# CrystalSixone/VLN-MAGIC

Hardware: AMD Instinct MI355X
Metric: trajectory-steps/sec (whole node), MAGIC-S R2R pretrain (higher is better)
Workload: dtype bf16

## Files before the change

profiles/micro/chain_timing.hip:

```cpp
#include "../../vln-magic_amd/csrc/chain.hip"
#include <cstdio>
GroupState& group_state() { static thread_local GroupState g = {}; return g; }
static void* dmalloc(size_t n, int fill) { void* p; hipMalloc(&p, n); hipMemset(p, fill, n); return p; }
int main(int argc, char** argv) {
  const int M = argc > 1 ? atoi(argv[1]) : 3840;
  ChainParams P; memset(&P, 0, sizeof(P));
  P.M = M; P.ld_in = CH; P.Np = 3 * CH; P.eps = 1e-12f;
  P.in = dmalloc((size_t)M * CH * 2, 0x11); P.res = dmalloc((size_t)M * CH * 2, 0x11);
  P.Wa = dmalloc(CH * CH * 2, 0x11); P.ba = (float*)dmalloc(CH * 4, 0); P.g1 = (float*)dmalloc(CH * 4, 0x3c); P.b1 = (float*)dmalloc(CH * 4, 0);
  P.W1 = dmalloc(CI * CH * 2, 0x11); P.bi = (float*)dmalloc(CI * 4, 0); P.W2 = dmalloc(CI * CH * 2, 0x11); P.bo2 = (float*)dmalloc(CH * 4, 0);
  P.g2 = (float*)dmalloc(CH * 4, 0x3c); P.b2 = (float*)dmalloc(CH * 4, 0); P.y2 = dmalloc((size_t)M * CH * 2, 0);
  P.Wp = dmalloc(3 * CH * CH * 2, 0x11); P.bp = (float*)dmalloc(3 * CH * 4, 0); P.proj = dmalloc((size_t)M * 3 * CH * 2, 0);
  hipEvent_t e0, e1; hipEventCreate(&e0); hipEventCreate(&e1);
  for (int rows = 32; rows <= 64; rows += 32)
  for (int variant = 0; variant < 3; ++variant) {
    magic_chain_tile_rows(rows);
    ChainParams Q = P;
    if (variant == 1) { Q.Wp = nullptr; }
    if (variant == 2) { Q.W1 = nullptr; Q.Np = CH; Q.y1 = Q.y2; }
    for (int it = 0; it < 3; ++it) magic_chain_fwd(DT_BF16, &Q, sizeof(Q), nullptr);
    hipDeviceSynchronize();
    hipEventRecord(e0);
    for (int it = 0; it < 20; ++it) magic_chain_fwd(DT_BF16, &Q, sizeof(Q), nullptr);
    hipEventRecord(e1); hipEventSynchronize(e1);
    float ms; hipEventElapsedTime(&ms, e0, e1);
    long long t[16]; hipMemcpyFromSymbol(t, HIP_SYMBOL(chain_ticks), sizeof(t));
    if (rows == 64) {
      printf("M %d rows 64 variant %d: %.1f us per launch; tile 0 (10 ns ticks): prologue %lld, stage-1 products %lld, LayerNorm 1 %lld, FFN (4 chunks) %lld, LayerNorm 2 %lld, y2 store + projection %lld, total %lld\n",
             M, variant, ms * 1000 / 20, t[1] - t[0], t[7] - t[1], t[2] - t[7], t[3] - t[2], t[4] - t[3], t[6] - t[4], t[6] - t[0]);
      continue;
    }
    printf("M %d variant %d (%s): %.1f us per launch; tile 0 (10 ns ticks): rows+params+ring prologue %lld, stage 1 %lld, 2a (8 chunks) %lld, 2b (8 chunks + LN) %lld, y2 store + 3 %lld, tail %lld, total %lld\n",
           M, variant, variant == 0 ? "full" : variant == 1 ? "no projection" : "mini", ms * 1000 / 20,
           t[1] - t[0], t[2] - t[1], t[3] - t[2], t[4] - t[3], t[5] - t[4], t[6] - t[5], t[6] - t[0]);
  }
  return 0;
}
```

vln-magic_amd/csrc/chain.hip:

```cpp
#include "enc_common.hpp"
#include "group.hpp"
#include <cstdlib>

#define CH 256
#define CI 1024
#define KP 264
#define KG 1032
#define CADDR(row, col, pitch) ((row) * (pitch) + (col))
#define CP 264
#define CG 1032

using ChainParams = magic_chain_params;

#define CRT 2
#define CROWS (16 * CRT)
#ifndef CNB
#define CNB 3
#endif

template <typename Hh>
__device__ __forceinline__ void chain_norm(f32x4 (&acc)[CRT][2], const float* sPar, const Hh* sR,
                                           float* red, Hh* sOut, const int nq, const float eps, const int w, const int lane) {
  const int g = lane >> 4, c16 = lane & 15;
  float bv[2], gv[2], btv[2];
#pragma unroll
  for (int ct = 0; ct < 2; ++ct) {
    const int col = (2 * w + ct) * 16 + c16;
    bv[ct] = sPar[col]; gv[ct] = sPar[CH + col]; btv[ct] = sPar[2 * CH + col];
  }
  float s[CRT][4];
#pragma unroll
  for (int rt = 0; rt < CRT; ++rt)
#pragma unroll
    for (int r = 0; r < 4; ++r) {
      const int row = rt * 16 + 4 * g + r;
#pragma unroll
      for (int ct = 0; ct < 2; ++ct) acc[rt][ct][r] += bv[ct] + to_f(sR[CADDR(row, (2 * w + ct) * 16 + c16, KP)]);
      s[rt][r] = row16_sum(acc[rt][0][r] + acc[rt][1][r]);
    }
  if (c16 == 0) {
#pragma unroll
    for (int rt = 0; rt < CRT; ++rt)
#pragma unroll
      for (int r = 0; r < 4; ++r) red[w * CROWS + rt * 16 + 4 * g + r] = s[rt][r];
  }
  __syncthreads();
  float mean[CRT][4];
#pragma unroll
  for (int rt = 0; rt < CRT; ++rt)
#pragma unroll
    for (int r = 0; r < 4; ++r) {
      float t = 0.f;
#pragma unroll
      for (int ww = 0; ww < NWAVE; ++ww) t += red[ww * CROWS + rt * 16 + 4 * g + r];
      mean[rt][r] = t * (1.0f / CH);
      const float d0 = acc[rt][0][r] - mean[rt][r], d1 = acc[rt][1][r] - mean[rt][r];
      s[rt][r] = row16_sum(d0 * d0 + d1 * d1);
    }
  if (c16 == 0) {
#pragma unroll
    for (int rt = 0; rt < CRT; ++rt)
#pragma unroll
      for (int r = 0; r < 4; ++r) red[NWAVE * CROWS + w * CROWS + rt * 16 + 4 * g + r] = s[rt][r];
  }
  __syncthreads();
#pragma unroll
  for (int rt = 0; rt < CRT; ++rt)
#pragma unroll
    for (int r = 0; r < 4; ++r) {
      const int rr = rt * 16 + 4 * g + r;
      float t = 0.f;
#pragma unroll
      for (int ww = 0; ww < NWAVE; ++ww) t += red[NWAVE * CROWS + ww * CROWS + rr];
      const float rstd = rsqrtf(t * (1.0f / CH) + eps);
#pragma unroll
      for (int ct = 0; ct < 2; ++ct)
        sOut[CADDR(rr, (2 * w + ct) * 16 + c16, KP)] = (rr < nq) ? from_f<Hh>((acc[rt][ct][r] - mean[rt][r]) * rstd * gv[ct] + btv[ct]) : (Hh)0.0f;
    }
}

template <typename Hh>
__device__ __forceinline__ void chain_rows_in(const Hh* src, long long ld, int nq, Hh* dst, int tid) {
  typedef __attribute__((ext_vector_type(4))) unsigned u4;
  for (int id = tid; id < CROWS * (CH / 8); id += NWAVE * 64) {
    const int r = id / (CH / 8), c = (id % (CH / 8)) * 8;
    const u4 v = r < nq ? *(const u4*)(src + r * ld + c) : (u4){0u, 0u, 0u, 0u};
    *(u4*)(dst + CADDR(r, c, KP)) = v;
  }
}

template <typename Hh> __device__ __forceinline__ h16x8<Hh> pfrag(const Hh* __restrict__ Wf, const int K, const int nt, const int ks, const int lane) {
  return *(const h16x8<Hh>*)(Wf + ((long long)(nt * (K >> 5) + ks) * 64 + lane) * 8);
}

template <typename Hh>
__device__ __forceinline__ void chain_load_chunk(h16x8<Hh> (&b)[8], const int cid, const ChainParams& p, const int w, const int lane, const int nct) {
  if (cid < 2) {
#pragma unroll
    for (int ks = 0; ks < 8; ++ks) b[ks] = pfrag((const Hh*)p.Wa, CH, 2 * w + cid, ks, lane);
  } else if (cid < 10) {
#pragma unroll
    for (int ks = 0; ks < 8; ++ks) b[ks] = pfrag((const Hh*)p.W1, CH, 8 * w + cid - 2, ks, lane);
  } else if (cid < 18) {
#pragma unroll
    for (int ks = 0; ks < 4; ++ks) {
      b[ks] = pfrag((const Hh*)p.W2, CI, 2 * w, 4 * (cid - 10) + ks, lane);
      b[4 + ks] = pfrag((const Hh*)p.W2, CI, 2 * w + 1, 4 * (cid - 10) + ks, lane);
    }
  } else {
    const Hh* Wq = p.Wp ? (const Hh*)p.Wp : (const Hh*)p.Wa;
    const int j = cid - 18, nt = p.Wp ? w * nct + (j < nct ? j : nct - 1) : 2 * w;
#pragma unroll
    for (int ks = 0; ks < 8; ++ks) b[ks] = pfrag(Wq, CH, nt, ks, lane);
  }
}

#ifdef CHAIN_TIMING
__device__ long long chain_ticks[16];
#define CH_MARK(i) do { if (tile == 0 && tid == 0) chain_ticks[i] = wall_clock64(); } while (0)
#else
#define CH_MARK(i)
#endif
template <typename Hh, bool FFN>
__device__ __forceinline__ void chain_body(const ChainParams& p, const int tile, unsigned char* smem) {
  Hh* sIn = (Hh*)smem;
  Hh* sRes = sIn + CROWS * KP;
  Hh* sY1 = sRes + CROWS * KP;
  Hh* sG = sY1 + CROWS * KP;
  float* red = (float*)(sG + CROWS * KG);
  Hh* sProj = sG;
  float* sPar = red + 2 * NWAVE * CROWS;
  const int tid = threadIdx.x, lane0 = tid & 63, w = __builtin_amdgcn_readfirstlane(tid >> 6);
  int lane = lane0;
  asm volatile("" : "+v"(lane));
  const int g = lane >> 4, c16 = lane & 15;
  const int row0 = tile * CROWS, nq = min(CROWS, p.M - row0);
  const int nct = p.Wp ? (p.Np >> 7) : 0;
  constexpr int NS = FFN ? 24 : 8;
#define SEQ(s) (FFN ? (s) : ((s) < 2 ? (s) : (s) + 16))
#define AHEAD(s) do { if ((s) + CNB - 1 < NS) chain_load_chunk<Hh>(ring[((s) + CNB - 1) % CNB], SEQ((s) + CNB - 1), p, w, lane, nct); } while (0)
  CH_MARK(0);
  chain_rows_in((const Hh*)p.inp + (long long)row0 * p.ld_in, p.ld_in, nq, sIn, tid);
  chain_rows_in((const Hh*)p.res + (long long)row0 * CH, CH, nq, sRes, tid);
  if (tid < CH) {
    sPar[tid] = p.ba[tid]; sPar[CH + tid] = p.g1[tid]; sPar[2 * CH + tid] = p.b1[tid];
    if (FFN) { sPar[3 * CH + tid] = p.bo2[tid]; sPar[4 * CH + tid] = p.g2[tid]; sPar[5 * CH + tid] = p.b2[tid]; }
  }
  if (FFN) { sPar[6 * CH + tid] = p.bi[tid]; sPar[6 * CH + 512 + tid] = p.bi[512 + tid]; }
  for (int i = tid; i < nct * 128; i += NWAVE * 64) sPar[6 * CH + CI + i] = p.bp[i];
  h16x8<Hh> ring[CNB][8];
#pragma unroll
  for (int s = 0; s < CNB - 1; ++s) chain_load_chunk<Hh>(ring[s], SEQ(s), p, w, lane, nct);
  __syncthreads();
  CH_MARK(1);
  {
    f32x4 acc[CRT][2];
#pragma unroll
    for (int rt = 0; rt < CRT; ++rt) { acc[rt][0] = (f32x4){0.f, 0.f, 0.f, 0.f}; acc[rt][1] = (f32x4){0.f, 0.f, 0.f, 0.f}; }
#pragma unroll
    for (int i = 0; i < 2; ++i) {
      AHEAD(i);
      KSTEP_FENCE();
#pragma unroll
      for (int ks = 0; ks < 8; ++ks)
#pragma unroll
        for (int rt = 0; rt < CRT; ++rt) acc[rt][i] = mfma16(frag_kc(sIn, KP, rt * 16, ks * 32, lane), ring[i % CNB][ks], acc[rt][i]);
      KSTEP_FENCE();
    }
    chain_norm(acc, sPar, sRes, red, sY1, nq, p.eps, w, lane);
  }
  __syncthreads();
  CH_MARK(2);
  if (p.y1) copy_out(sY1, KP, (Hh*)p.y1 + (long long)row0 * CH, CH, nq, CH, tid);
  const Hh* sLast = sY1;
  if constexpr (FFN) {
    {
#pragma unroll
      for (int ct = 0; ct < 8; ++ct) {
        AHEAD(2 + ct);
        const int col = (8 * w + ct) * 16 + c16;
        const float bfc = sPar[6 * CH + col];
        KSTEP_FENCE();
        f32x4 acc[CRT];
#pragma unroll
        for (int rt = 0; rt < CRT; ++rt) acc[rt] = (f32x4){0.f, 0.f, 0.f, 0.f};
#pragma unroll
        for (int ks = 0; ks < 8; ++ks)
#pragma unroll
          for (int rt = 0; rt < CRT; ++rt) acc[rt] = mfma16(frag_kc(sY1, KP, rt * 16, ks * 32, lane), ring[(2 + ct) % CNB][ks], acc[rt]);
#pragma unroll
        for (int rt = 0; rt < CRT; ++rt)
#pragma unroll
          for (int r = 0; r < 4; ++r) sG[CADDR(rt * 16 + 4 * g + r, col, KG)] = from_f<Hh>(gelu_fast(acc[rt][r] + bfc));
        KSTEP_FENCE();
      }
    }
    __syncthreads();
    CH_MARK(3);
    {
      f32x4 acc[CRT][2];
#pragma unroll
      for (int rt = 0; rt < CRT; ++rt) { acc[rt][0] = (f32x4){0.f, 0.f, 0.f, 0.f}; acc[rt][1] = (f32x4){0.f, 0.f, 0.f, 0.f}; }
#pragma unroll
      for (int ch = 0; ch < 8; ++ch) {
        AHEAD(10 + ch);
        KSTEP_FENCE();
#pragma unroll
        for (int ks = 0; ks < 4; ++ks)
#pragma unroll
          for (int rt = 0; rt < CRT; ++rt) {
            const h16x8<Hh> a = frag_kc(sG, KG, rt * 16, (4 * ch + ks) * 32, lane);
            acc[rt][0] = mfma16(a, ring[(10 + ch) % CNB][ks], acc[rt][0]);
            acc[rt][1] = mfma16(a, ring[(10 + ch) % CNB][4 + ks], acc[rt][1]);
          }
        KSTEP_FENCE();
      }
      chain_norm(acc, sPar + 3 * CH, sY1, red, sIn, nq, p.eps, w, lane);
    }
    __syncthreads();
    CH_MARK(4);
    copy_out(sIn, KP, (Hh*)p.y2 + (long long)row0 * CH, CH, nq, CH, tid);
    sLast = sIn;
  }
  if (nct) {
    constexpr int S3 = FFN ? 18 : 2;
    const int pp = p.Np + 8;
#pragma unroll
    for (int j = 0; j < 6; ++j) {
      AHEAD(S3 + j);
      if (j < nct) {
        const int tile_n = w * nct + j;
        const float bpv = sPar[6 * CH + CI + tile_n * 16 + c16];
        KSTEP_FENCE();
        f32x4 acc[CRT];
#pragma unroll
        for (int rt = 0; rt < CRT; ++rt) acc[rt] = (f32x4){0.f, 0.f, 0.f, 0.f};
#pragma unroll
        for (int ks = 0; ks < 8; ++ks)
#pragma unroll
          for (int rt = 0; rt < CRT; ++rt) acc[rt] = mfma16(frag_kc(sLast, KP, rt * 16, ks * 32, lane), ring[(S3 + j) % CNB][ks], acc[rt]);
#pragma unroll
        for (int rt = 0; rt < CRT; ++rt)
#pragma unroll
          for (int r = 0; r < 4; ++r) sProj[(rt * 16 + 4 * g + r) * pp + tile_n * 16 + c16] = from_f<Hh>(acc[rt][r] + bpv);
      }
      KSTEP_FENCE();
    }
    __syncthreads();
    CH_MARK(5);
    copy_out(sProj, pp, (Hh*)p.proj + (long long)row0 * p.Np, p.Np, nq, p.Np, tid);
  }
  CH_MARK(6);
#undef SEQ
#undef AHEAD
}

struct ChainPair { ChainParams p[2]; int split; };
#ifndef CHAIN_ATTR
#define CHAIN_ATTR
#endif
template <typename Hh>
__global__ __launch_bounds__(512) CHAIN_ATTR void chain_fwd_kernel(ChainPair pr) {
  extern __shared__ __attribute__((aligned(16))) unsigned char chain_smem[];
  const int which = (int)blockIdx.x < pr.split ? 0 : 1;
  const ChainParams& p = pr.p[which];
  const int tile = which ? blockIdx.x - pr.split : blockIdx.x;
  if (p.W1) chain_body<Hh, true>(p, tile, chain_smem);
  else chain_body<Hh, false>(p, tile, chain_smem);
}


typedef __attribute__((ext_vector_type(16))) float f32x16;
__device__ __forceinline__ f32x16 mfma32(bf16x8 a, bf16x8 b, f32x16 c) { return __builtin_amdgcn_mfma_f32_32x32x16_bf16(a, b, c, 0, 0, 0); }
__device__ __forceinline__ f32x16 mfma32(f16x8 a, f16x8 b, f32x16 c) { return __builtin_amdgcn_mfma_f32_32x32x16_f16(a, b, c, 0, 0, 0); }
template <typename Hh> __device__ __forceinline__ h16x8<Hh> lfrag32(const Hh* s, int pitch, int row0, int k0, int lane) {
  return *(const h16x8<Hh>*)(s + (row0 + (lane & 31)) * pitch + k0 + 8 * (lane >> 5));
}
template <typename Hh> __device__ __forceinline__ h16x8<Hh> pfrag32(const Hh* __restrict__ Wf, const int K, const int NT, const int KS, const int lane) {
  const int nt16 = 2 * NT + ((lane >> 4) & 1), l2 = (lane & 15) + 16 * (2 * (KS & 1) + (lane >> 5));
  return *(const h16x8<Hh>*)(Wf + ((long long)(nt16 * (K >> 5) + (KS >> 1)) * 64 + l2) * 8);
}
#define C6ROWS 64
#define C6RT 2
#define C6NB 3
template <typename Hh>
__device__ __forceinline__ void chain64_load_chunk(h16x8<Hh> (&b)[8], const int cid, const ChainParams& p, const int w, const int lane, const int nj) {
  if (cid < 2) {
#pragma unroll
    for (int ks = 0; ks < 8; ++ks) b[ks] = pfrag32((const Hh*)p.Wa, CH, w, 8 * cid + ks, lane);
  } else if (cid < 18) {
    const int c = (cid - 2) >> 2, q = (cid - 2) & 3;
    if (q < 2) {
#pragma unroll
      for (int ks = 0; ks < 8; ++ks) b[ks] = pfrag32((const Hh*)p.W1, CH, 8 * c + w, 8 * q + ks, lane);
    } else {
#pragma unroll
      for (int ks = 0; ks < 8; ++ks) b[ks] = pfrag32((const Hh*)p.W2, CI, w, 16 * c + 8 * (q - 2) + ks, lane);
    }
  } else {
    const Hh* Wq = p.Wp ? (const Hh*)p.Wp : (const Hh*)p.Wa;
    const int j = (cid - 18) >> 1, hf = (cid - 18) & 1, nt = p.Wp ? 8 * (j < nj ? j : nj - 1) + w : w;
#pragma unroll
    for (int ks = 0; ks < 8; ++ks) b[ks] = pfrag32(Wq, CH, nt, 8 * hf + ks, lane);
  }
}
template <typename Hh>
__device__ __forceinline__ void chain64_norm(f32x16 (&acc)[C6RT], const float* sPar, const Hh* sR, float* red, Hh* sOut, const float eps,
                                             const int w, const int lane) {
  const int col = 32 * w + (lane & 31), h = lane >> 5, sub = (lane >> 4) & 1;
  const float bv = sPar[col], gv = sPar[CH + col], btv = sPar[2 * CH + col];
  float* part1 = red;
  float* part2 = red + 16 * C6ROWS;
  float* stat = red + 32 * C6ROWS + w * C6ROWS;
#pragma unroll
  for (int rt = 0; rt < C6RT; ++rt)
#pragma unroll
    for (int i = 0; i < 16; ++i) {
      const int row = rt * 32 + (i & 3) + 8 * (i >> 2) + 4 * h;
      acc[rt][i] += bv + to_f(sR[row * CP + col]);
      const float s = row16_sum(acc[rt][i]);
      if ((lane & 15) == 0) part1[(2 * w + sub) * C6ROWS + row] = s;
    }
  __syncthreads();
  {
    float t = 0.f;
#pragma unroll
    for (int q = 0; q < 16; ++q) t += part1[q * C6ROWS + lane];
    stat[lane] = t * (1.0f / CH);
  }
  wave_lds_sync();
#pragma unroll
  for (int rt = 0; rt < C6RT; ++rt)
#pragma unroll
    for (int i4 = 0; i4 < 4; ++i4) {
      const f32x4 m4 = *(const f32x4*)(stat + rt * 32 + 8 * i4 + 4 * h);
#pragma unroll
      for (int r = 0; r < 4; ++r) {
        const int i = 4 * i4 + r, row = rt * 32 + r + 8 * i4 + 4 * h;
        acc[rt][i] -= m4[r];
        const float s = row16_sum(acc[rt][i] * acc[rt][i]);
        if ((lane & 15) == 0) part2[(2 * w + sub) * C6ROWS + row] = s;
      }
    }
  __syncthreads();
  {
    float t = 0.f;
#pragma unroll
    for (int q = 0; q < 16; ++q) t += part2[q * C6ROWS + lane];
    wave_lds_sync();
    stat[lane] = rsqrtf(t * (1.0f / CH) + eps);
  }
  wave_lds_sync();
#pragma unroll
  for (int rt = 0; rt < C6RT; ++rt)
#pragma unroll
    for (int i4 = 0; i4 < 4; ++i4) {
      const f32x4 r4 = *(const f32x4*)(stat + rt * 32 + 8 * i4 + 4 * h);
#pragma unroll
      for (int r = 0; r < 4; ++r) {
        const int i = 4 * i4 + r, row = rt * 32 + r + 8 * i4 + 4 * h;
        sOut[row * CP + col] = from_f<Hh>(acc[rt][i] * r4[r] * gv + btv);
      }
    }
}
template <typename Hh>
__device__ __forceinline__ void chain64_rows_in(const Hh* src, long long ld, int nq, Hh* dst, int tid) {
  typedef __attribute__((ext_vector_type(4))) unsigned u4;
  for (int id = tid; id < C6ROWS * (CH / 8); id += NWAVE * 64) {
    const int r = id / (CH / 8), c = (id % (CH / 8)) * 8;
    const u4 v = r < nq ? *(const u4*)(src + r * ld + c) : (u4){0u, 0u, 0u, 0u};
    *(u4*)(dst + r * CP + c) = v;
  }
}
template <typename Hh, bool FFN>
__device__ __forceinline__ void chain64_body(const ChainParams& p, const int tile, unsigned char* smem) {
  Hh* sIn = (Hh*)smem;
  Hh* sRes = sIn + C6ROWS * CP;
  Hh* sY1 = sRes + C6ROWS * CP;
  Hh* sG = sY1 + C6ROWS * CP;
  float* red = (float*)(sG + C6ROWS * CP);
  float* sPar = red + 40 * C6ROWS;
  const int tid = threadIdx.x, lane0 = tid & 63, w = __builtin_amdgcn_readfirstlane(tid >> 6);
  int lane = lane0;
  asm volatile("" : "+v"(lane));
  const int h = lane >> 5, c32 = lane & 31;
  const int row0 = tile * C6ROWS, nq = min(C6ROWS, p.M - row0);
  const int nj = p.Wp ? (p.Np >> 8) : 0;
  constexpr int NS = FFN ? 24 : 8;
#define SEQ6(s) (FFN ? (s) : ((s) < 2 ? (s) : (s) + 16))
#define AHEAD6(s) do { if ((s) + C6NB - 1 < NS) chain64_load_chunk<Hh>(ring[((s) + C6NB - 1) % C6NB], SEQ6((s) + C6NB - 1), p, w, lane, nj); } while (0)
  CH_MARK(0);
  chain64_rows_in((const Hh*)p.inp + (long long)row0 * p.ld_in, p.ld_in, nq, sIn, tid);
  chain64_rows_in((const Hh*)p.res + (long long)row0 * CH, CH, nq, sRes, tid);
  if (tid < CH) {
    sPar[tid] = p.ba[tid]; sPar[CH + tid] = p.g1[tid]; sPar[2 * CH + tid] = p.b1[tid];
    if (FFN) { sPar[3 * CH + tid] = p.bo2[tid]; sPar[4 * CH + tid] = p.g2[tid]; sPar[5 * CH + tid] = p.b2[tid]; }
  }
  if (FFN) { sPar[6 * CH + tid] = p.bi[tid]; sPar[6 * CH + 512 + tid] = p.bi[512 + tid]; }
  for (int i = tid; i < nj * 256; i += NWAVE * 64) sPar[6 * CH + CI + i] = p.bp[i];
  h16x8<Hh> ring[C6NB][8];
#pragma unroll
  for (int s = 0; s < C6NB - 1; ++s) chain64_load_chunk<Hh>(ring[s], SEQ6(s), p, w, lane, nj);
  __syncthreads();
  CH_MARK(1);
  {
    f32x16 acc[C6RT];
#pragma unroll
    for (int rt = 0; rt < C6RT; ++rt)
#pragma unroll
      for (int i = 0; i < 16; ++i) acc[rt][i] = 0.f;
#pragma unroll
    for (int i = 0; i < 2; ++i) {
      AHEAD6(i);
      KSTEP_FENCE();
#pragma unroll
      for (int ks = 0; ks < 8; ++ks)
#pragma unroll
        for (int rt = 0; rt < C6RT; ++rt) acc[rt] = mfma32(lfrag32(sIn, CP, rt * 32, (8 * i + ks) * 16, lane), ring[i % C6NB][ks], acc[rt]);
      KSTEP_FENCE();
    }
    CH_MARK(7);
    chain64_norm(acc, sPar, sRes, red, sY1, p.eps, w, lane);
  }
  __syncthreads();
  CH_MARK(2);
  if (p.y1) copy_out(sY1, CP, (Hh*)p.y1 + (long long)row0 * CH, CH, nq, CH, tid);
  const Hh* sLast = sY1;
  if constexpr (FFN) {
    f32x16 acc2[C6RT];
#pragma unroll
    for (int rt = 0; rt < C6RT; ++rt)
#pragma unroll
      for (int i = 0; i < 16; ++i) acc2[rt][i] = 0.f;
#pragma unroll
    for (int c = 0; c < 4; ++c) {
      Hh* gbuf = (c & 1) ? sRes : sG;
      {
        f32x16 acc[C6RT];
#pragma unroll
        for (int rt = 0; rt < C6RT; ++rt)
#pragma unroll
          for (int i = 0; i < 16; ++i) acc[rt][i] = 0.f;
        const float bfc = sPar[6 * CH + 256 * c + 32 * w + c32];
#pragma unroll
        for (int q = 0; q < 2; ++q) {
          AHEAD6(2 + 4 * c + q);
          KSTEP_FENCE();
#pragma unroll
          for (int ks = 0; ks < 8; ++ks)
#pragma unroll
            for (int rt = 0; rt < C6RT; ++rt) acc[rt] = mfma32(lfrag32(sY1, CP, rt * 32, (8 * q + ks) * 16, lane), ring[(2 + 4 * c + q) % C6NB][ks], acc[rt]);
          KSTEP_FENCE();
        }
#pragma unroll
        for (int rt = 0; rt < C6RT; ++rt)
#pragma unroll
          for (int i = 0; i < 16; ++i)
            gbuf[(rt * 32 + (i & 3) + 8 * (i >> 2) + 4 * h) * CP + 32 * w + c32] = from_f<Hh>(gelu_fast(acc[rt][i] + bfc));
      }
      __syncthreads();
#pragma unroll
      for (int q = 0; q < 2; ++q) {
        AHEAD6(4 + 4 * c + q);
        KSTEP_FENCE();
#pragma unroll
        for (int ks = 0; ks < 8; ++ks)
#pragma unroll
          for (int rt = 0; rt < C6RT; ++rt) acc2[rt] = mfma32(lfrag32(gbuf, CP, rt * 32, (8 * q + ks) * 16, lane), ring[(4 + 4 * c + q) % C6NB][ks], acc2[rt]);
        KSTEP_FENCE();
      }
    }
    CH_MARK(3);
    chain64_norm(acc2, sPar + 3 * CH, sY1, red, sIn, p.eps, w, lane);
    __syncthreads();
    CH_MARK(4);
    copy_out(sIn, CP, (Hh*)p.y2 + (long long)row0 * CH, CH, nq, CH, tid);
    sLast = sIn;
  }
  if (nj) {
    constexpr int S3 = FFN ? 18 : 2;
#pragma unroll
    for (int j = 0; j < 3; ++j) {
      f32x16 acc[C6RT];
#pragma unroll
      for (int rt = 0; rt < C6RT; ++rt)
#pragma unroll
        for (int i = 0; i < 16; ++i) acc[rt][i] = 0.f;
#pragma unroll
      for (int q = 0; q < 2; ++q) {
        AHEAD6(S3 + 2 * j + q);
        KSTEP_FENCE();
        if (j < nj) {
#pragma unroll
          for (int ks = 0; ks < 8; ++ks)
#pragma unroll
            for (int rt = 0; rt < C6RT; ++rt) acc[rt] = mfma32(lfrag32(sLast, CP, rt * 32, (8 * q + ks) * 16, lane), ring[(S3 + 2 * j + q) % C6NB][ks], acc[rt]);
        }
        KSTEP_FENCE();
      }
      if (j < nj) {
        const float bpv = sPar[6 * CH + CI + 256 * j + 32 * w + c32];
        Hh* pbuf = (j & 1) ? sRes : sG;
#pragma unroll
        for (int rt = 0; rt < C6RT; ++rt)
#pragma unroll
          for (int i = 0; i < 16; ++i)
            pbuf[(rt * 32 + (i & 3) + 8 * (i >> 2) + 4 * h) * CP + 32 * w + c32] = from_f<Hh>(acc[rt][i] + bpv);
        __syncthreads();
        copy_out(pbuf, CP, (Hh*)p.proj + (long long)row0 * p.Np + 256 * j, p.Np, nq, 256, tid);
      }
    }
  }
  CH_MARK(6);
#undef SEQ6
#undef AHEAD6
}
template <typename Hh>
__global__ __launch_bounds__(512) void chain64_fwd_kernel(ChainPair pr) {
  extern __shared__ __attribute__((aligned(16))) unsigned char chain_smem[];
  const int which = (int)blockIdx.x < pr.split ? 0 : 1;
  const ChainParams& p = pr.p[which];
  const int tile = which ? blockIdx.x - pr.split : blockIdx.x;
  if (p.W1) chain64_body<Hh, true>(p, tile, chain_smem);
  else chain64_body<Hh, false>(p, tile, chain_smem);
}
static size_t chain64_lds_bytes() { return (size_t)(4 * C6ROWS * CP) * 2 + (40 * C6ROWS + 6 * CH + CI + 3 * CH) * sizeof(float); }

static size_t chain_lds_bytes() { return (size_t)(3 * CROWS * KP + CROWS * KG) * 2 + (2 * NWAVE * CROWS + 6 * CH + CI + 3 * CH) * sizeof(float); }

static bool chain_valid(const ChainParams& p) {
  if (p.M <= 0 || !p.inp || !p.res || !p.Wa || !p.ba || !p.g1 || !p.b1 || p.ld_in < CH || (p.ld_in & 7)) return false;
  if (p.W1 && (!p.bi || !p.W2 || !p.bo2 || !p.g2 || !p.b2 || !p.y2)) return false;
  if (p.Wp && (!p.bp || !p.proj || (p.Np != CH && p.Np != 2 * CH && p.Np != 3 * CH))) return false;
  if (!p.W1 && !p.y1 && !p.Wp) return false;
  return true;
}

static int chain_rows_cfg = 0;
extern "C" int magic_chain_tile_rows(int rows) {
  if (!chain_rows_cfg) { const char* e = getenv("MAGIC_CHAIN_ROWS"); const int v = e ? atoi(e) : 1; chain_rows_cfg = (v == 32 || v == 64) ? v : 1; }
  if (rows == 1 || rows == 32 || rows == 64) chain_rows_cfg = rows;
  else if (rows != 0) return MAGIC_ERR_ARG;
  return chain_rows_cfg;
}

int launch_chain(int dtype, int variant, const void* pa_, const void* pb_, hipStream_t st) {
  (void)variant;
  ChainPair pr;
  pr.p[0] = *(const ChainParams*)pa_;
  pr.p[1] = pb_ ? *(const ChainParams*)pb_ : pr.p[0];
  static int min_tiles = -1;
  if (min_tiles < 0) {
    const char* e = getenv("MAGIC_CHAIN_64_MIN_TILES");
    hipDeviceProp_t pr; int d = 0; (void)hipGetDevice(&d);
    min_tiles = e ? atoi(e) : ((hipGetDeviceProperties(&pr, d) == hipSuccess ? pr.multiProcessorCount : 256) + 1);
  }
  const int t32 = (pr.p[0].M + 31) / 32 + (pb_ ? (pr.p[1].M + 31) / 32 : 0);
  const int cfg = magic_chain_tile_rows(0);
  const int rows = cfg == 1 ? (t32 >= min_tiles ? 64 : 32) : cfg;
  const int ta = (pr.p[0].M + rows - 1) / rows, tb = pb_ ? (pr.p[1].M + rows - 1) / rows : 0;
  pr.split = ta;
  static bool attr_done[3] = {false, false, false};
  if (!attr_done[dtype == DT_BF16 ? DT_BF16 : DT_F16]) {
    DISPATCH_H(dtype, hipFuncSetAttribute((const void*)chain_fwd_kernel<TY>, hipFuncAttributeMaxDynamicSharedMemorySize, (int)chain_lds_bytes());
                      hipFuncSetAttribute((const void*)chain64_fwd_kernel<TY>, hipFuncAttributeMaxDynamicSharedMemorySize, (int)chain64_lds_bytes()));
    attr_done[dtype == DT_BF16 ? DT_BF16 : DT_F16] = true;
  }
  const size_t lds = rows == 64 ? chain64_lds_bytes() : chain_lds_bytes();
  DISPATCH_H(dtype, if (rows == 64) hipLaunchKernelGGL(chain64_fwd_kernel<TY>, dim3(ta + tb), dim3(512), lds, st, pr);
                    else hipLaunchKernelGGL(chain_fwd_kernel<TY>, dim3(ta + tb), dim3(512), lds, st, pr));
  return launch_status();
}

#define FSP_MAX 160
struct FSpans { long long off[FSP_MAX]; int rows[FSP_MAX]; int cols[FSP_MAX]; int blk0[FSP_MAX + 1]; int n; };
__global__ __launch_bounds__(256) void pack_frag_spans_kernel(const unsigned short* __restrict__ src, unsigned short* __restrict__ dst, FSpans t) {
  typedef __attribute__((ext_vector_type(8))) unsigned short u16x8;
  const int id = blockIdx.x;
  int s = 0;
  for (int i = 1; i < t.n; ++i) s += (id >= t.blk0[i]) ? 1 : 0;
  const int C = t.cols[s];
  const long long chunk = (long long)(id - t.blk0[s]) * 256 + threadIdx.x;
  const int l = (int)(chunk & 63);
  const long long frag = chunk >> 6;
  const int kpr = C >> 5, nt = (int)(frag / kpr), ks = (int)(frag % kpr);
  const unsigned short* a = src + t.off[s] + (long long)(16 * nt + (l & 15)) * C + 32 * ks + 8 * (l >> 4);
  *(u16x8*)(dst + t.off[s] + chunk * 8) = *(const u16x8*)a;
}
extern "C" int magic_pack_frag_spans(const void* src, void* dst, int n, const long long* offs, const int* rows, const int* cols, void* stream) {
  if (!src || !dst || n < 0 || (n && (!offs || !rows || !cols)) || ((uintptr_t)src & 15) || ((uintptr_t)dst & 15)) return MAGIC_ERR_ARG;
  for (int i = 0; i < n; ++i)
    if (rows[i] <= 0 || cols[i] <= 0 || rows[i] % 16 || cols[i] % 32 || ((long long)rows[i] * cols[i]) % 2048 || offs[i] % 8) return MAGIC_ERR_ARG;
  for (int base = 0; base < n; base += FSP_MAX) {
    FSpans t;
    t.n = n - base < FSP_MAX ? n - base : FSP_MAX;
    int blocks = 0;
    for (int i = 0; i < t.n; ++i) {
      t.off[i] = offs[base + i]; t.rows[i] = rows[base + i]; t.cols[i] = cols[base + i];
      t.blk0[i] = blocks;
      blocks += (int)(((long long)rows[base + i] * cols[base + i]) / 2048);
    }
    t.blk0[t.n] = blocks;
    hipLaunchKernelGGL(pack_frag_spans_kernel, dim3(blocks), dim3(256), 0, (hipStream_t)stream, (const unsigned short*)src, (unsigned short*)dst, t);
  }
  return launch_status();
}

struct LSpans { long long off[FSP_MAX]; int rows[FSP_MAX]; int cols[FSP_MAX]; int flags[FSP_MAX]; int tile0[FSP_MAX + 1]; int n; };
__global__ __launch_bounds__(256) void layout_spans_kernel(const unsigned short* __restrict__ src, unsigned short* __restrict__ dst_f,
                                                           unsigned short* __restrict__ dst_tf, LSpans t) {
  typedef __attribute__((ext_vector_type(8))) unsigned short u16x8;
  __shared__ unsigned short tile[64][72];
  const int id = blockIdx.x;
  int s = 0;
  for (int i = 1; i < t.n; ++i) s += (id >= t.tile0[i]) ? 1 : 0;
  const int local = id - t.tile0[s], R = t.rows[s], C = t.cols[s], fl = t.flags[s];
  const int tc = C / 64, r0 = (local / tc) * 64, c0 = (local % tc) * 64;
  const unsigned short* a = src + t.off[s];
#pragma unroll
  for (int it = 0; it < 2; ++it) {
    const int ch = threadIdx.x + it * 256, r = ch >> 3, c = (ch & 7) * 8;
    const u16x8 v = *(const u16x8*)(a + (long long)(r0 + r) * C + c0 + c);
    *(u16x8*)&tile[r][c] = v;
    if (fl & 1) {
      const int nt = (r0 + r) >> 4, rr = (r0 + r) & 15, ks = (c0 + c) >> 5, g = ((c0 + c) & 31) >> 3;
      *(u16x8*)(dst_f + t.off[s] + ((long long)(nt * (C >> 5) + ks) * 64 + g * 16 + rr) * 8) = v;
    }
  }
  if (!(fl & 2)) return;
  __syncthreads();
#pragma unroll
  for (int it = 0; it < 2; ++it) {
    const int ch = threadIdx.x + it * 256, l = ch & 63, fr = ch >> 6, i = fr >> 1, j = fr & 1, g = l >> 4, nn = l & 15;
    u16x8 v;
#pragma unroll
    for (int e = 0; e < 8; ++e) v[e] = tile[32 * j + 8 * g + e][16 * i + nn];
    const int nt = (c0 >> 4) + i, ks = (r0 >> 5) + j;
    *(u16x8*)(dst_tf + t.off[s] + ((long long)(nt * (R >> 5) + ks) * 64 + l) * 8) = v;
  }
}
extern "C" int magic_layout_spans(const void* src, void* dst_f, void* dst_tf, int n, const long long* offs, const int* rows, const int* cols,
                                  const int* flags, void* stream) {
  if (!src || n < 0 || (n && (!offs || !rows || !cols || !flags)) || ((uintptr_t)src & 15) || ((uintptr_t)dst_f & 15) || ((uintptr_t)dst_tf & 15)) return MAGIC_ERR_ARG;
  for (int i = 0; i < n; ++i) {
    if (rows[i] <= 0 || cols[i] <= 0 || rows[i] % 64 || cols[i] % 64 || offs[i] % 8 || !(flags[i] & 3)) return MAGIC_ERR_ARG;
    if (((flags[i] & 1) && !dst_f) || ((flags[i] & 2) && !dst_tf)) return MAGIC_ERR_ARG;
  }
  for (int base = 0; base < n; base += FSP_MAX) {
    LSpans t;
    t.n = n - base < FSP_MAX ? n - base : FSP_MAX;
    int tiles = 0;
    for (int i = 0; i < t.n; ++i) {
      t.off[i] = offs[base + i]; t.rows[i] = rows[base + i]; t.cols[i] = cols[base + i]; t.flags[i] = flags[base + i];
      t.tile0[i] = tiles;
      tiles += (rows[base + i] / 64) * (cols[base + i] / 64);
    }
    t.tile0[t.n] = tiles;
    hipLaunchKernelGGL(layout_spans_kernel, dim3(tiles), dim3(256), 0, (hipStream_t)stream, (const unsigned short*)src, (unsigned short*)dst_f,
                       (unsigned short*)dst_tf, t);
  }
  return launch_status();
}

extern "C" int magic_chain_supported(int dtype, int H, int I) { return dtype_is16(dtype) && H == CH && I == CI; }

extern "C" int magic_chain_fwd(int dtype, const void* params, int nbytes, void* stream) {
  if (!params || nbytes != (int)sizeof(ChainParams) || !dtype_is16(dtype)) return MAGIC_ERR_ARG;
  ChainParams p;
  memcpy(&p, params, sizeof(p));
  if (!chain_valid(p)) return MAGIC_ERR_ARG;
  if (group_record(KIND_CHAIN, dtype, 0, &p, sizeof(p))) return MAGIC_OK;
  return launch_chain(dtype, 0, &p, nullptr, (hipStream_t)stream);
}
```

vln-magic_amd/csrc/common.hpp:

```cpp
#pragma once
#include <hip/hip_runtime.h>
#include <stdint.h>
#include "../../include/magic_hip.h"

typedef __bf16 bf16;
typedef __attribute__((ext_vector_type(8))) __bf16 bf16x8;
typedef __attribute__((ext_vector_type(4))) __bf16 bf16x4;
typedef __attribute__((ext_vector_type(4))) float f32x4;
typedef _Float16 f16;
typedef __attribute__((ext_vector_type(8))) _Float16 f16x8;
typedef __attribute__((ext_vector_type(4))) _Float16 f16x4;
typedef __attribute__((ext_vector_type(4))) short s16x4;

#define DT_F32 0
#define DT_BF16 1
#define DT_F16 2
static inline bool dtype_ok(int dt) { return dt == DT_F32 || dt == DT_BF16 || dt == DT_F16; }
static inline bool dtype_is16(int dt) { return dt == DT_BF16 || dt == DT_F16; }

#define DISPATCH_T(dtype, ...)                                                        \
  do {                                                                                \
    if ((dtype) == DT_BF16) { typedef bf16 TY; __VA_ARGS__; }                          \
    else if ((dtype) == DT_F16) { typedef f16 TY; __VA_ARGS__; }                       \
    else { typedef float TY; __VA_ARGS__; }                                           \
  } while (0)
#define DISPATCH_H(dtype, ...)                                                        \
  do {                                                                                \
    if ((dtype) == DT_BF16) { typedef bf16 TY; __VA_ARGS__; }                          \
    else { typedef f16 TY; __VA_ARGS__; }                                             \
  } while (0)
#define DISPATCH_NIT(dtype, H, F)                                                                                       \
  DISPATCH_T(dtype, if ((H) == 128) F(TY, 1); else if ((H) == 256) F(TY, 2); else if ((H) == 384) F(TY, 3);              \
                    else if ((H) == 768) F(TY, 6); else return MAGIC_ERR_UNSUPPORTED)
#define DISPATCH_I2(v, A, B, ...)                                                     \
  do {                                                                                \
    if ((v) == (A)) { constexpr int IV = (A); __VA_ARGS__; }                           \
    else { constexpr int IV = (B); __VA_ARGS__; }                                     \
  } while (0)
#define DISPATCH_I3(v, A, B, C, ...)                                                  \
  do {                                                                                \
    if ((v) == (A)) { constexpr int IV = (A); __VA_ARGS__; }                           \
    else if ((v) == (B)) { constexpr int IV = (B); __VA_ARGS__; }                      \
    else { constexpr int IV = (C); __VA_ARGS__; }                                     \
  } while (0)

#define WAVE 64

__device__ __forceinline__ float to_f(float x) { return x; }
__device__ __forceinline__ float to_f(bf16 x) { return (float)x; }
__device__ __forceinline__ float to_f(f16 x) { return (float)x; }
template <typename T> __device__ __forceinline__ T from_f(float x);
template <> __device__ __forceinline__ float from_f<float>(float x) { return x; }
template <> __device__ __forceinline__ bf16 from_f<bf16>(float x) { return (bf16)x; }
template <> __device__ __forceinline__ f16 from_f<f16>(float x) { return (f16)x; }

template <typename Hh> struct H16;
template <> struct H16<bf16> { typedef bf16x8 v8; typedef bf16x4 v4; };
template <> struct H16<f16> { typedef f16x8 v8; typedef f16x4 v4; };
template <typename Hh> using h16x8 = typename H16<Hh>::v8;
template <typename Hh> using h16x4 = typename H16<Hh>::v4;
__device__ __forceinline__ f32x4 mfma16(bf16x8 a, bf16x8 b, f32x4 c) { return __builtin_amdgcn_mfma_f32_16x16x32_bf16(a, b, c, 0, 0, 0); }
__device__ __forceinline__ f32x4 mfma16(f16x8 a, f16x8 b, f32x4 c) { return __builtin_amdgcn_mfma_f32_16x16x32_f16(a, b, c, 0, 0, 0); }
__device__ __forceinline__ bf16x4 lds_tr4(const bf16* p) {
  typedef bf16x4 __attribute__((address_space(3))) * lds4;
  return __builtin_amdgcn_ds_read_tr16_b64_v4bf16((lds4)p);
}
__device__ __forceinline__ f16x4 lds_tr4(const f16* p) {
  typedef s16x4 __attribute__((address_space(3))) * lds4;
  return __builtin_bit_cast(f16x4, __builtin_amdgcn_ds_read_tr16_b64_v4i16((lds4)p));
}
template <typename Hh> __device__ __forceinline__ h16x8<Hh> lds_tr8(const Hh* p, int pitch4) {
  const h16x4<Hh> lo = lds_tr4(p), hi = lds_tr4(p + pitch4);
  return __builtin_shufflevector(lo, hi, 0, 1, 2, 3, 4, 5, 6, 7);
}
__device__ __forceinline__ f32x4 mfma16(float a, float b, f32x4 c) { return __builtin_amdgcn_mfma_f32_16x16x4f32(a, b, c, 0, 0, 0); }
template <typename Hh> __device__ __forceinline__ h16x8<Hh> frag_kc(const Hh* s, int pitch, int row0, int k0, int lane) {
  return *(const h16x8<Hh>*)(s + (row0 + (lane & 15)) * pitch + k0 + 8 * (lane >> 4));
}
template <typename Hh> __device__ __forceinline__ h16x8<Hh> frag_oc(const Hh* s, int pitch, int row0, int k0, int lane) {
  const int g = lane >> 4, q = (lane & 15) >> 2, pp = lane & 3;
  return lds_tr8(s + (k0 + 8 * g + q) * pitch + row0 + 4 * pp, 4 * pitch);
}
__device__ __forceinline__ float frag_kc(const float* s, int pitch, int row0, int k0, int lane) { return s[(row0 + (lane & 15)) * pitch + k0 + (lane >> 4)]; }
__device__ __forceinline__ float frag_oc(const float* s, int pitch, int row0, int k0, int lane) { return s[(k0 + (lane >> 4)) * pitch + row0 + (lane & 15)]; }

template <typename T> struct RowVecT { typedef T type __attribute__((ext_vector_type(16 / sizeof(T)))); };
template <typename T> using rowvec = typename RowVecT<T>::type;
template <typename T> struct RowImg {
  T* s; int pitch;
  const T* src; int ld;
  int nvalid, cvalid;
  int cpr, nchunk;
};
template <int NIT, typename T>
__device__ __forceinline__ void stage_issue(rowvec<T> (&reg)[NIT], const RowImg<T>& im, const int it0, const int tid, const int nthr) {
  constexpr int VE = 16 / sizeof(T);
#pragma unroll
  for (int it = 0; it < NIT; ++it) {
    const int id = tid + (it0 + it) * nthr, r = id / im.cpr, c = (id - r * im.cpr) * VE;
#pragma unroll
    for (int e = 0; e < VE; ++e) reg[it][e] = (T)0.0f;
    if (id < im.nchunk && r < im.nvalid && c < im.cvalid) reg[it] = *(const rowvec<T>*)(im.src + c + __mul24(r, im.ld));
  }
}
template <int NIT, typename T>
__device__ __forceinline__ void stage_store(const rowvec<T> (&reg)[NIT], const RowImg<T>& im, const int it0, const int tid, const int nthr) {
  constexpr int VE = 16 / sizeof(T);
#pragma unroll
  for (int it = 0; it < NIT; ++it) {
    const int id = tid + (it0 + it) * nthr, r = id / im.cpr, c = (id - r * im.cpr) * VE;
    if (id < im.nchunk) *(rowvec<T>*)(im.s + r * im.pitch + c) = reg[it];
  }
}

template <int CTRL> __device__ __forceinline__ float dpp_mov(float v) {
  return __int_as_float(__builtin_amdgcn_update_dpp(0, __float_as_int(v), CTRL, 0xF, 0xF, true));
}
#define DPP_QUAD_XOR1 0xB1
#define DPP_QUAD_XOR2 0x4E
#define DPP_ROW_HALF_MIRROR 0x141
#define DPP_ROW_MIRROR 0x140
__device__ __forceinline__ float row16_sum(float v) {
  v += dpp_mov<DPP_QUAD_XOR1>(v);
  v += dpp_mov<DPP_QUAD_XOR2>(v);
  v += dpp_mov<DPP_ROW_HALF_MIRROR>(v);
  v += dpp_mov<DPP_ROW_MIRROR>(v);
  return v;
}
__device__ __forceinline__ float row16_max(float v) {
  v = fmaxf(v, dpp_mov<DPP_QUAD_XOR1>(v));
  v = fmaxf(v, dpp_mov<DPP_QUAD_XOR2>(v));
  v = fmaxf(v, dpp_mov<DPP_ROW_HALF_MIRROR>(v));
  v = fmaxf(v, dpp_mov<DPP_ROW_MIRROR>(v));
  return v;
}
__device__ __forceinline__ float lane_bcast(float v, int lane) { return __int_as_float(__builtin_amdgcn_readlane(__float_as_int(v), lane)); }
__device__ __forceinline__ float wave_sum(float v) {
  v = row16_sum(v);
  return (lane_bcast(v, 0) + lane_bcast(v, 16)) + (lane_bcast(v, 32) + lane_bcast(v, 48));
}
__device__ __forceinline__ float wave_max(float v) {
  v = row16_max(v);
  return fmaxf(fmaxf(lane_bcast(v, 0), lane_bcast(v, 16)), fmaxf(lane_bcast(v, 32), lane_bcast(v, 48)));
}
__device__ __forceinline__ int wave_min_i(int v) {
#pragma unroll
  for (int d = 1; d < WAVE; d <<= 1) v = min(v, __shfl_xor(v, d));
  return v;
}
template <typename T> __device__ __forceinline__ T wave_scan_sum(T v, int lane) {
#pragma unroll
  for (int d = 1; d < WAVE; d <<= 1) {
    const T o = __shfl_up(v, d);
    if (lane >= d) v += o;
  }
  return v;
}

__device__ __forceinline__ float gelu_f(float x) { return 0.5f * x * (1.0f + erff(x * 0.70710678118654752f)); }
__device__ __forceinline__ float dgelu_f(float x) {
  float cdf = 0.5f * (1.0f + erff(x * 0.70710678118654752f));
  float pdf = 0.39894228040143268f * __expf(-0.5f * x * x);
  return cdf + x * pdf;
}

using DropDesc = magic_drop_desc;
struct DropState { unsigned ka, kb, thr; float scale; bool on; };
__device__ __forceinline__ DropState drop_init(const DropDesc& d) {
  DropState s;
  s.on = d.seed != nullptr && d.p > 0.f;
  s.ka = 0; s.kb = 0; s.thr = 0; s.scale = 1.f;
  if (s.on) {
    s.ka = d.seed[0] ^ (d.site * 0x9E3779B1u);
    s.kb = d.seed[1] + d.site * 0x85EBCA77u;
    s.thr = (unsigned)((double)d.p * 4294967296.0);
    s.scale = 1.0f / (1.0f - d.p);
  }
  return s;
}
__device__ __forceinline__ float drop_mul(const DropState& s, unsigned idx) {
  unsigned x = (idx ^ s.ka) + s.kb;
  x ^= x >> 16; x *= 0x85EBCA6Bu; x ^= x >> 13; x *= 0xC2B2AE35u; x ^= x >> 16;
  return x >= s.thr ? s.scale : 0.f;
}
static inline bool drop_args_ok(const void* seed, float p) { return p >= 0.f && p < 1.f && (p == 0.f || seed != nullptr); }

const float* seed_scale_get();

static inline int launch_status() {
  hipError_t e = hipGetLastError();
  return e == hipSuccess ? MAGIC_OK : MAGIC_ERR_LAUNCH;
}

#define CSJ_MAX 96
struct ColsumJobs { const float* part[CSJ_MAX]; float* dst[CSJ_MAX]; int nblk[CSJ_MAX]; int n; };
__device__ __forceinline__ void colsum_body(const ColsumJobs& js, const int j, const int H, float* red) {
  const int t = threadIdx.x, c = t % H, grp = t / H, ngrp = blockDim.x / H;
  const float* part = js.part[j];
  const int nb = js.nblk[j];
  float s0 = 0.f, s1 = 0.f, s2 = 0.f, s3 = 0.f;
  if (grp < ngrp) {
    int b = grp;
    for (; b + 3 * ngrp < nb; b += 4 * ngrp) {
      s0 += part[(long long)b * H + c]; s1 += part[(long long)(b + ngrp) * H + c];
      s2 += part[(long long)(b + 2 * ngrp) * H + c]; s3 += part[(long long)(b + 3 * ngrp) * H + c];
    }
    for (; b < nb; b += ngrp) s0 += part[(long long)b * H + c];
  }
  red[t] = (s0 + s1) + (s2 + s3);
  __syncthreads();
  if (grp == 0) {
    float v = 0.f;
    for (int g2 = 0; g2 < ngrp; ++g2) v += red[g2 * H + c];
    js.dst[j][c] += v;
  }
}
```

vln-magic_amd/csrc/encoder.hip:

```cpp
#include "enc_common.hpp"
#include <cstdlib>
#include <cstring>

template <typename Hh> struct EncLayerT {
  const Hh* Wqkv; const float* bqkv;
  const Hh* Wo; const float* bo; const float* g1; const float* be1;
  const Hh* W1; const float* bi;
  const Hh* W2; const float* bo2; const float* g2; const float* be2;
  Hh *qkv, *P, *Pd, *ctx, *a, *z, *g, *out;
  float *rstd_a, *rstd_o;
  unsigned site_attn, site_ao, site_out, pad_;
};
template <typename Hh> struct EncSegT { const Hh* x; const unsigned char* kmask; int nsamp, N, ldp, nlayers; EncLayerT<Hh> L[6]; };
template <typename Hh> struct EncParamsT {
  EncSegT<Hh> seg[2]; int nseg; float p_attn, p_hidden, eps, scale; const unsigned* seed;
  unsigned* sync; int sync_words, pad2_;
};
typedef EncParamsT<bf16> EncParams; typedef EncSegT<bf16> EncSeg; typedef EncLayerT<bf16> EncLayer;
#define F(f) ABI_VIEW(EncLayer, magic_enc_layer, f)
F(Wqkv) F(bqkv) F(Wo) F(bo) F(g1) F(be1) F(W1) F(bi) F(W2) F(bo2) F(g2) F(be2) F(qkv) F(P) F(Pd) F(ctx) F(a) F(z) F(g) F(out) F(rstd_a) F(rstd_o)
F(site_attn) F(site_ao) F(site_out) F(pad_)
#undef F
#define F(f) ABI_VIEW(EncSeg, magic_enc_seg, f)
F(x) F(kmask) F(nsamp) F(N) F(ldp) F(nlayers) F(L)
#undef F
#define F(f) ABI_VIEW(EncParams, magic_enc_params, f)
F(seg) F(nseg) F(p_attn) F(p_hidden) F(eps) F(scale) F(seed) F(sync) F(sync_words) F(pad2_)
#undef F

template <int NRT, int RSTR, typename Hh>
__device__ __forceinline__ void add_norm(f32x4 (&acc)[NRT], const float bv, const float gv, const float btv, const Hh* sRes,
                                         float* red, Hh* sOut, float* gRstd, int N, long long row_base, float eps,
                                         const DropState& ds, int w, int lane) {
  const int g = lane >> 4, c16 = lane & 15, col = w * 16 + c16;
  float s[NRT][4];
#pragma unroll
  for (int i = 0; i < NRT; ++i)
#pragma unroll
    for (int r = 0; r < 4; ++r) {
      const int row = i * 16 + 4 * g + r;
      float v = acc[i][r] + bv;
      if (ds.on) v *= drop_mul(ds, (unsigned)((row_base + row) * EH + col));
      v += to_f(sRes[row * XS + col]);
      acc[i][r] = v;
      s[i][r] = row16_sum(v);
    }
  if (c16 == 0) {
#pragma unroll
    for (int i = 0; i < NRT; ++i)
#pragma unroll
      for (int r = 0; r < 4; ++r) red[w * RSTR + i * 16 + 4 * g + r] = s[i][r];
  }
  __syncthreads();
  float mean[NRT][4];
#pragma unroll
  for (int i = 0; i < NRT; ++i)
#pragma unroll
    for (int r = 0; r < 4; ++r) {
      const int rr = i * 16 + 4 * g + r;
      float t = 0.f;
#pragma unroll
      for (int ww = 0; ww < NWAVE; ++ww) t += red[ww * RSTR + rr];
      mean[i][r] = t * (1.0f / EH);
    }
  __syncthreads();
#pragma unroll
  for (int i = 0; i < NRT; ++i)
#pragma unroll
    for (int r = 0; r < 4; ++r) {
      const float d = acc[i][r] - mean[i][r];
      s[i][r] = row16_sum(d * d);
    }
  if (c16 == 0) {
#pragma unroll
    for (int i = 0; i < NRT; ++i)
#pragma unroll
      for (int r = 0; r < 4; ++r) red[w * RSTR + i * 16 + 4 * g + r] = s[i][r];
  }
  __syncthreads();
#pragma unroll
  for (int i = 0; i < NRT; ++i)
#pragma unroll
    for (int r = 0; r < 4; ++r) {
      const int rr = i * 16 + 4 * g + r;
      float t = 0.f;
#pragma unroll
      for (int ww = 0; ww < NWAVE; ++ww) t += red[ww * RSTR + rr];
      const float rstd = rsqrtf(t * (1.0f / EH) + eps);
      const Hh y = from_f<Hh>((acc[i][r] - mean[i][r]) * rstd * gv + btv);
      sOut[rr * XS + col] = (rr < N) ? y : (Hh)0.0f;
      if (rr < N && w == 0 && c16 == 0) gRstd[row_base + rr] = rstd;
    }
}

#ifdef ENC_TIMING
__device__ long long enc_ticks[2][16];
#define ENC_MARK(i) do { if (samp == 0 && tid == 0) enc_ticks[&sg == &p.seg[0] ? 0 : 1][i] = wall_clock64(); } while (0)
#else
#define ENC_MARK(i)
#endif

__device__ unsigned magic_enc_starts;
__device__ long long magic_enc_start_tick;
__device__ __forceinline__ void enc_mark_start() {
  if (blockIdx.x == gridDim.x - 1 && threadIdx.x == 0) {
    __hip_atomic_store(&magic_enc_start_tick, (long long)wall_clock64(), __ATOMIC_RELAXED, __HIP_MEMORY_SCOPE_AGENT);
    __hip_atomic_fetch_add(&magic_enc_starts, 1u, __ATOMIC_RELAXED, __HIP_MEMORY_SCOPE_AGENT);
  }
}

template <int NRT> struct EncLay {
  static constexpr bool COMPACT = NRT <= 3;
  static constexpr int RA = COMPACT ? 48 : MAXROWS;
  static constexpr int KR = COMPACT ? 49 : KROWS;
  static constexpr int PW = COMPACT ? 72 : PSW;
};
template <typename Hh> __device__ __forceinline__ h16x8<Hh> tfrag_z(const Hh* s, int pitch, int n0, int k0, int lane, int kmax, int zrow) {
  const int g = lane >> 4, q = (lane & 15) >> 2, pp = lane & 3;
  int r0 = k0 + 8 * g + q, r1 = r0 + 4;
  r0 = r0 < kmax ? r0 : zrow; r1 = r1 < kmax ? r1 : zrow;
  const h16x4<Hh> lo = lds_tr4(s + r0 * pitch + n0 + 4 * pp), hi = lds_tr4(s + r1 * pitch + n0 + 4 * pp);
  return __builtin_shufflevector(lo, hi, 0, 1, 2, 3, 4, 5, 6, 7);
}

template <int NRT, typename Hh>
__device__ __forceinline__ void enc_body(const EncParamsT<Hh>& p, const EncSegT<Hh>& sg, const int samp, unsigned char* smem) {
  typedef EncLay<NRT> LY;
  constexpr int RA = LY::RA, KR = LY::KR, PW = LY::PW;
  Hh* sX = (Hh*)smem;
  Hh* sA = sX + RA * XS;
  Hh* sQKV = sA + RA * XS;
  Hh* sP = sQKV + KR * QS;
  Hh* sG = sQKV;
  float* red = LY::COMPACT ? (float*)(sQKV + RA * GS) : (float*)(sP + NWAVE * 16 * PSW);
  const int tid = threadIdx.x, lane0 = tid & 63, w = __builtin_amdgcn_readfirstlane(tid >> 6);
  const int N = sg.N, ldp = sg.ldp;
  const int NKP = (N + 31) / 32 * 32;
  const long long row_base = (long long)samp * N;
  constexpr int ROWS = NRT * 16;

  {
    const Hh* x = sg.x + row_base * EH;
    for (int id = tid; id < ROWS * (EH / 8); id += NWAVE * 64) {
      const int r = id / (EH / 8), c = (id % (EH / 8)) * 8;
      h16x8<Hh> v;
#pragma unroll
      for (int e = 0; e < 8; ++e) v[e] = (Hh)0.0f;
      if (r < N) v = *(const h16x8<Hh>*)(x + (long long)r * EH + c);
      *(h16x8<Hh>*)(sX + r * XS + c) = v;
    }
  }
  DropDesc dd;
  dd.seed = p.seed;
  float kbias[NRT];
#pragma unroll
  for (int j = 0; j < NRT; ++j) {
    const int key = j * 16 + (lane0 & 15);
    kbias[j] = (key < N && sg.kmask && !sg.kmask[(long long)samp * N + key]) ? -10000.0f : 0.f;
  }
  for (int l = 0; l < sg.nlayers; ++l) {
    const EncLayerT<Hh>& L = sg.L[l];
    int lane = lane0;
    asm volatile("" : "+v"(lane));
    const int g = lane >> 4, c16 = lane & 15;
    ENC_MARK(0);
    float pb_qkv[3], pb_ffn[4];
#pragma unroll
    for (int ct = 0; ct < 3; ++ct) pb_qkv[ct] = L.bqkv[(3 * w + ct) * 16 + c16];
#pragma unroll
    for (int ct = 0; ct < 4; ++ct) pb_ffn[ct] = L.bi[(4 * w + ct) * 16 + c16];
    const float pb_o = L.bo[w * 16 + c16], pg_1 = L.g1[w * 16 + c16], pe_1 = L.be1[w * 16 + c16];
    const float pb_2 = L.bo2[w * 16 + c16], pg_2 = L.g2[w * 16 + c16], pe_2 = L.be2[w * 16 + c16];
    h16x8<Hh> bw[3][4];
#pragma unroll
    for (int ct = 0; ct < 3; ++ct)
#pragma unroll
      for (int ks = 0; ks < 4; ++ks) bw[ct][ks] = gfrag(L.Wqkv, EH, (3 * w + ct) * 16, ks * 32, lane);
    for (int id = tid; id < (KR - (LY::COMPACT ? 48 : ROWS)) * (384 / 8); id += NWAVE * 64) {
      const int r = (LY::COMPACT ? 48 : ROWS) + id / 48, c = (id % 48) * 8;
      h16x8<Hh> zv;
#pragma unroll
      for (int e = 0; e < 8; ++e) zv[e] = (Hh)0.0f;
      *(h16x8<Hh>*)(sQKV + r * QS + c) = zv;
    }
    __syncthreads();
    ENC_MARK(1);
    {
      f32x4 acc[NRT][3];
#pragma unroll
      for (int i = 0; i < NRT; ++i)
#pragma unroll
        for (int ct = 0; ct < 3; ++ct) acc[i][ct] = (f32x4){0.f, 0.f, 0.f, 0.f};
#pragma unroll
      for (int ks = 0; ks < 4; ++ks) {
#pragma unroll
        for (int i = 0; i < NRT; ++i) {
          const h16x8<Hh> a = frag_kc(sX, XS, i * 16, ks * 32, lane);
#pragma unroll
          for (int ct = 0; ct < 3; ++ct) acc[i][ct] = mfma16(a, bw[ct][ks], acc[i][ct]);
        }
        KSTEP_FENCE();
      }
#pragma unroll
      for (int ct = 0; ct < 3; ++ct) {
        const int col = (3 * w + ct) * 16 + c16;
        const float bv = pb_qkv[ct];
#pragma unroll
        for (int i = 0; i < NRT; ++i)
#pragma unroll
          for (int r = 0; r < 4; ++r) sQKV[(i * 16 + 4 * g + r) * QS + col] = from_f<Hh>(acc[i][ct][r] + bv);
      }
    }
    h16x8<Hh> wo[4];
#pragma unroll
    for (int ks = 0; ks < 4; ++ks) wo[ks] = gfrag(L.Wo, EH, w * 16, ks * 32, lane);
    __syncthreads();
    copy_out(sQKV, QS, L.qkv + row_base * 3 * EH, 3 * EH, N, 3 * EH, tid);
    ENC_MARK(2);
    h16x8<Hh> w1[4][4];
#pragma unroll
    for (int ct = 0; ct < (NRT > 4 ? 2 : 4); ++ct)
#pragma unroll
      for (int ks = 0; ks < 4; ++ks) w1[ct][ks] = gfrag(L.W1, EH, (4 * w + ct) * 16, ks * 32, lane);
    dd.site = L.site_attn; dd.p = p.p_attn;
    const DropState dsa = drop_init(dd);
    Hh* sPw = sP + w * 16 * PW;
    for (int u = w; u < ENH * NRT; u += NWAVE) {
      const int h = u / NRT, rt = u % NRT;
      f32x4 sc[NRT];
#pragma unroll
      for (int j = 0; j < NRT; ++j) sc[j] = (f32x4){0.f, 0.f, 0.f, 0.f};
#pragma unroll
      for (int ks = 0; ks < 2; ++ks) {
        const h16x8<Hh> a = frag_kc(sQKV, QS, rt * 16, h * EHD + ks * 32, lane);
#pragma unroll
        for (int j = 0; j < NRT; ++j) sc[j] = mfma16(a, frag_kc(sQKV, QS, j * 16, EH + h * EHD + ks * 32, lane), sc[j]);
      }
      float mx[4] = {-3.0e38f, -3.0e38f, -3.0e38f, -3.0e38f};
#pragma unroll
      for (int j = 0; j < NRT; ++j) {
        const int key = j * 16 + c16;
        const bool kv = key < N;
        const float mb = kbias[j];
#pragma unroll
        for (int r = 0; r < 4; ++r) {
          float x = sc[j][r] * p.scale + mb;
          x = kv ? x : -3.0e38f;
          sc[j][r] = x; mx[r] = fmaxf(mx[r], x);
        }
      }
      float sum[4];
#pragma unroll
      for (int r = 0; r < 4; ++r) { mx[r] = row16_max(mx[r]); sum[r] = 0.f; }
#pragma unroll
      for (int j = 0; j < NRT; ++j) {
        const bool kv = (j * 16 + c16) < N;
#pragma unroll
        for (int r = 0; r < 4; ++r) { const float e = kv ? __expf(sc[j][r] - mx[r]) : 0.f; sc[j][r] = e; sum[r] += e; }
      }
#pragma unroll
      for (int r = 0; r < 4; ++r) sum[r] = 1.0f / row16_sum(sum[r]);
#pragma unroll
      for (int j = 0; j < NRT; ++j)
#pragma unroll
        for (int r = 0; r < 4; ++r) sPw[(4 * g + r) * PW + j * 16 + c16] = from_f<Hh>(sc[j][r] * sum[r]);
      if (NRT * 16 < NKP) {
        for (int id = lane; id < 16 * (NKP - NRT * 16); id += 64) {
          const int r = id / (NKP - NRT * 16), c = NRT * 16 + id % (NKP - NRT * 16);
          sPw[r * PW + c] = (Hh)0.0f;
        }
      }
      wave_lds_sync();
      const int nq = min(16, N - rt * 16);
      {
        Hh* Pg = L.P + (((long long)samp * ENH + h) * N + rt * 16) * ldp;
        const int cpr = ldp / 8;
        for (int id = lane; id < nq * cpr; id += 64) {
          const int r = id / cpr, c = (id % cpr) * 8;
          *(h16x8<Hh>*)(Pg + (long long)r * ldp + c) = *(const h16x8<Hh>*)(sPw + r * PW + c);
        }
      }
      if (dsa.on) {
#pragma unroll
        for (int j = 0; j < NRT; ++j) {
          const int key = j * 16 + c16;
#pragma unroll
          for (int r = 0; r < 4; ++r) {
            const int ql = 4 * g + r;
            const unsigned idx = (unsigned)(((((long long)samp * ENH + h) * N + rt * 16 + ql) * N) + key);
            const float m = (ql < nq && key < N) ? drop_mul(dsa, idx) : 0.f;
            sPw[ql * PW + key] = from_f<Hh>(sc[j][r] * sum[r] * m);
          }
        }
        wave_lds_sync();
        if (L.Pd) {
          Hh* Pg = L.Pd + (((long long)samp * ENH + h) * N + rt * 16) * ldp;
          const int cpr = ldp / 8;
          for (int id = lane; id < nq * cpr; id += 64) {
            const int r = id / cpr, c = (id % cpr) * 8;
            *(h16x8<Hh>*)(Pg + (long long)r * ldp + c) = *(const h16x8<Hh>*)(sPw + r * PW + c);
          }
        }
      }
      f32x4 o[4];
#pragma unroll
      for (int jd = 0; jd < 4; ++jd) o[jd] = (f32x4){0.f, 0.f, 0.f, 0.f};
      for (int ks = 0; ks < NKP / 32; ++ks) {
        const h16x8<Hh> a = frag_kc(sPw, PW, 0, ks * 32, lane);
#pragma unroll
        for (int jd = 0; jd < 4; ++jd) o[jd] = mfma16(a, LY::COMPACT ? tfrag_z(sQKV + 2 * EH + h * EHD, QS, jd * 16, ks * 32, lane, 48, 48)
                                    : frag_oc(sQKV + 2 * EH + h * EHD, QS, jd * 16, ks * 32, lane), o[jd]);
      }
#pragma unroll
      for (int jd = 0; jd < 4; ++jd)
#pragma unroll
        for (int r = 0; r < 4; ++r) sA[(rt * 16 + 4 * g + r) * XS + h * EHD + jd * 16 + c16] = from_f<Hh>(o[jd][r]);
    }
    ENC_MARK(3);
    if (NRT > 4) {
#pragma unroll
      for (int ct = 2; ct < 4; ++ct)
#pragma unroll
        for (int ks = 0; ks < 4; ++ks) w1[ct][ks] = gfrag(L.W1, EH, (4 * w + ct) * 16, ks * 32, lane);
    }
    __syncthreads();
    copy_out(sA, XS, L.ctx + row_base * EH, EH, N, EH, tid);
    ENC_MARK(4);
    {
      f32x4 acc[NRT];
#pragma unroll
      for (int i = 0; i < NRT; ++i) acc[i] = (f32x4){0.f, 0.f, 0.f, 0.f};
#pragma unroll
      for (int ks = 0; ks < 4; ++ks) {
#pragma unroll
        for (int i = 0; i < NRT; ++i) acc[i] = mfma16(frag_kc(sA, XS, i * 16, ks * 32, lane), wo[ks], acc[i]);
        KSTEP_FENCE();
      }
      dd.site = L.site_ao; dd.p = p.p_hidden;
      const DropState dsh = drop_init(dd);
      add_norm<NRT, RA>(acc, pb_o, pg_1, pe_1, sX, red, sA, L.rstd_a, N, row_base, p.eps, dsh, w, lane);
    }
    __syncthreads();
    copy_out(sA, XS, L.a + row_base * EH, EH, N, EH, tid);
    ENC_MARK(5);
    h16x8<Hh> w2[16];
    {
      f32x4 acc[NRT][4];
#pragma unroll
      for (int i = 0; i < NRT; ++i)
#pragma unroll
        for (int ct = 0; ct < 4; ++ct) acc[i][ct] = (f32x4){0.f, 0.f, 0.f, 0.f};
#pragma unroll
      for (int ks = 0; ks < 4; ++ks) {
#pragma unroll
        for (int i = 0; i < NRT; ++i) {
          const h16x8<Hh> a = frag_kc(sA, XS, i * 16, ks * 32, lane);
#pragma unroll
          for (int ct = 0; ct < 4; ++ct) acc[i][ct] = mfma16(a, w1[ct][ks], acc[i][ct]);
        }
        KSTEP_FENCE();
      }
#pragma unroll
      for (int ks = 0; ks < 16; ++ks) w2[ks] = gfrag(L.W2, EI, w * 16, ks * 32, lane);
#pragma unroll
      for (int ct = 0; ct < 4; ++ct) {
        const int col = (4 * w + ct) * 16 + c16;
#pragma unroll
        for (int i = 0; i < NRT; ++i)
#pragma unroll
          for (int r = 0; r < 4; ++r) {
            acc[i][ct][r] += pb_ffn[ct];
            sG[(i * 16 + 4 * g + r) * GS + col] = from_f<Hh>(acc[i][ct][r]);
          }
      }
      __syncthreads();
      copy_out(sG, GS, L.z + row_base * EI, EI, N, EI, tid);
#pragma unroll
      for (int ct = 0; ct < 4; ++ct)
#pragma unroll
        for (int i = 0; i < NRT; ++i)
#pragma unroll
          for (int r = 0; r < 4; ++r) acc[i][ct][r] = gelu_fast(acc[i][ct][r]);
      __syncthreads();
#pragma unroll
      for (int ct = 0; ct < 4; ++ct) {
        const int col = (4 * w + ct) * 16 + c16;
#pragma unroll
        for (int i = 0; i < NRT; ++i)
#pragma unroll
          for (int r = 0; r < 4; ++r) sG[(i * 16 + 4 * g + r) * GS + col] = from_f<Hh>(acc[i][ct][r]);
      }
    }
    ENC_MARK(6);
    __syncthreads();
    copy_out(sG, GS, L.g + row_base * EI, EI, N, EI, tid);
    ENC_MARK(7);
    {
      f32x4 acc[NRT];
#pragma unroll
      for (int i = 0; i < NRT; ++i) acc[i] = (f32x4){0.f, 0.f, 0.f, 0.f};
#pragma unroll
      for (int ks = 0; ks < 16; ++ks) {
#pragma unroll
        for (int i = 0; i < NRT; ++i) acc[i] = mfma16(frag_kc(sG, GS, i * 16, ks * 32, lane), w2[ks], acc[i]);
        if ((ks & 1) == 1) KSTEP_FENCE();
      }
      dd.site = L.site_out; dd.p = p.p_hidden;
      const DropState dsh = drop_init(dd);
      add_norm<NRT, RA>(acc, pb_2, pg_2, pe_2, sA, red, sX, L.rstd_o, N, row_base, p.eps, dsh, w, lane);
    }
    __syncthreads();
    copy_out(sX, XS, L.out + row_base * EH, EH, N, EH, tid);
    ENC_MARK(8);
  }
}

template <typename Hh>
__global__ __launch_bounds__(512) void encoder_fwd_kernel(EncParamsT<Hh> p) {
  enc_mark_start();
  extern __shared__ __attribute__((aligned(16))) unsigned char enc_smem[];
  int b = blockIdx.x, s = 0;
  if (b >= p.seg[0].nsamp) { b -= p.seg[0].nsamp; s = 1; }
  const EncSegT<Hh>& sg = p.seg[s];
  const int nrt = max(2, (sg.N + 15) / 16);
  switch (nrt) {
    case 2: enc_body<2>(p, sg, b, enc_smem); break;
    case 3: enc_body<3>(p, sg, b, enc_smem); break;
    case 4: enc_body<4>(p, sg, b, enc_smem); break;
    default: enc_body<5>(p, sg, b, enc_smem); break;
  }
}

#define RS_ZROW 80
#define RS_SS 84
#define RS_PP 104
#define RS_SPIN_MAX (1u << 21)
typedef __attribute__((ext_vector_type(4))) unsigned u32x4;
typedef __attribute__((address_space(1))) unsigned gu32_t;
__device__ unsigned magic_enc_gave_up;
__device__ __forceinline__ void enc_give_up(gu32_t* err) {
  __hip_atomic_store(err, 1u, __ATOMIC_RELAXED, __HIP_MEMORY_SCOPE_AGENT);
  __hip_atomic_fetch_add(&magic_enc_gave_up, 1u, __ATOMIC_RELAXED, __HIP_MEMORY_SCOPE_AGENT);
}

template <typename Hh> __device__ __forceinline__ h16x8<Hh> tfrag_clamp(const Hh* s, int pitch, int n0, int k0, int lane, int kmax) {
  const int g = lane >> 4, q = (lane & 15) >> 2, pp = lane & 3;
  int r0 = k0 + 8 * g + q, r1 = r0 + 4;
  r0 = r0 < kmax ? r0 : RS_ZROW; r1 = r1 < kmax ? r1 : RS_ZROW;
  const h16x4<Hh> lo = lds_tr4(s + r0 * pitch + n0 + 4 * pp), hi = lds_tr4(s + r1 * pitch + n0 + 4 * pp);
  return __builtin_shufflevector(lo, hi, 0, 1, 2, 3, 4, 5, 6, 7);
}

template <typename Hh>
__device__ __forceinline__ void add_norm16(f32x4& acc, const float bv, const float gv, const float btv, const Hh* sRes, float* red, Hh* sOut,
                                           float* gRstd, const int nq, const long long row0, const float eps, const DropState& ds, const int w, const int lane) {
  const int g = lane >> 4, c16 = lane & 15, col = w * 16 + c16;
  float s[4];
#pragma unroll
  for (int r = 0; r < 4; ++r) {
    const int row = 4 * g + r;
    float v = acc[r] + bv;
    if (ds.on) v *= drop_mul(ds, (unsigned)((row0 + row) * EH + col));
    v += to_f(sRes[row * XS + col]);
    acc[r] = v;
    s[r] = row16_sum(v);
  }
  if (c16 == 0) {
#pragma unroll
    for (int r = 0; r < 4; ++r) red[w * 16 + 4 * g + r] = s[r];
  }
  __syncthreads();
  float mean[4];
#pragma unroll
  for (int r = 0; r < 4; ++r) {
    float t = 0.f;
#pragma unroll
    for (int ww = 0; ww < NWAVE; ++ww) t += red[ww * 16 + 4 * g + r];
    mean[r] = t * (1.0f / EH);
    const float d = acc[r] - mean[r];
    s[r] = row16_sum(d * d);
  }
  if (c16 == 0) {
#pragma unroll
    for (int r = 0; r < 4; ++r) red[128 + w * 16 + 4 * g + r] = s[r];
  }
  __syncthreads();
#pragma unroll
  for (int r = 0; r < 4; ++r) {
    const int rr = 4 * g + r;
    float t = 0.f;
#pragma unroll
    for (int ww = 0; ww < NWAVE; ++ww) t += red[128 + ww * 16 + rr];
    const float rstd = rsqrtf(t * (1.0f / EH) + eps);
    const Hh y = from_f<Hh>((acc[r] - mean[r]) * rstd * gv + btv);
    sOut[rr * XS + col] = (rr < nq) ? y : (Hh)0.0f;
    if (rr < nq && w == 0 && c16 == 0) gRstd[row0 + rr] = rstd;
  }
}

template <bool SC1, typename Hh>
__device__ __forceinline__ void copy_tile(const Hh* s, int pitch, Hh* g, int ldg, int rows, int cols, int tid) {
  const int cpr = cols / 8;
  if constexpr (SC1) {
    const auto rsrc = __builtin_amdgcn_make_buffer_rsrc((void*)g, 0, rows * ldg * 2, 0x00020000);
    for (int id = tid; id < rows * cpr; id += NWAVE * 64) {
      const int r = id / cpr, c = (id % cpr) * 8;
      __builtin_amdgcn_raw_buffer_store_b128(*(const u32x4*)(s + r * pitch + c), rsrc, (r * ldg + c) * 2, 0, 16);
    }
  } else {
    for (int id = tid; id < rows * cpr; id += NWAVE * 64) {
      const int r = id / cpr, c = (id % cpr) * 8;
      *(h16x8<Hh>*)(g + (long long)r * ldg + c) = *(const h16x8<Hh>*)(s + r * pitch + c);
    }
  }
}

#ifdef ENC_TIMING
__device__ long long rs_ticks[8][16];
#define RS_MARK(i) do { if (samp == 0 && tile == 0 && tid == 0 && &sg == &p.seg[0]) rs_ticks[l][i] = wall_clock64(); } while (0)
#else
#define RS_MARK(i)
#endif
template <int NRT, typename Hh>
__device__ __forceinline__ void enc_rs_body(const EncParamsT<Hh>& p, const EncSegT<Hh>& sg, const int samp, const int tile, unsigned* cnt,
                                            unsigned* err, unsigned char* smem) {
  Hh* sK = (Hh*)smem;
  Hh* sV = sK + 80 * XS;
  Hh* sU = sV + 81 * XS;
  Hh* sX = sU;
  float* sS = (float*)sU;
  Hh* sPd = sU + 2 * 16 * RS_SS * 2;
  Hh* sG = sU;
  Hh* sZ = sK;
  Hh* sQ = sU + 80 * XS;
  Hh* sO = sQ + 16 * XS;
  Hh* sA = sO + 16 * XS;
  float* red = (float*)(sA + 16 * XS);
  const int tid = threadIdx.x, lane0 = tid & 63, w = __builtin_amdgcn_readfirstlane(tid >> 6);
  const int N = sg.N, ldp = sg.ldp;
  const int NKP = (N + 31) / 32 * 32;
  const long long row_base = (long long)samp * N;
  const int r0 = tile * 16, nq = min(16, N - r0);
  const long long row0 = row_base + r0;
  if (tid < XS / 8) {
    h16x8<Hh> zv;
#pragma unroll
    for (int e = 0; e < 8; ++e) zv[e] = (Hh)0.0f;
    *(h16x8<Hh>*)(sV + RS_ZROW * XS + tid * 8) = zv;
  }
  DropDesc dd;
  dd.seed = p.seed;
  float kbias[NRT];
#pragma unroll
  for (int j = 0; j < NRT; ++j) {
    const int key = j * 16 + (lane0 & 15);
    kbias[j] = (key < N && sg.kmask && !sg.kmask[(long long)samp * N + key]) ? -10000.0f : 0.f;
  }
  for (int l = 0; l < sg.nlayers; ++l) {
    const EncLayerT<Hh>& L = sg.L[l];
    int lane = lane0;
    asm volatile("" : "+v"(lane));
    const int g = lane >> 4, c16 = lane & 15;
    RS_MARK(0);
    const float pb_q = L.bqkv[w * 16 + c16], pb_kv0 = L.bqkv[EH + (2 * w) * 16 + c16], pb_kv1 = L.bqkv[EH + (2 * w + 1) * 16 + c16];
    float pb_ffn[4];
#pragma unroll
    for (int ct = 0; ct < 4; ++ct) pb_ffn[ct] = L.bi[(4 * w + ct) * 16 + c16];
    const float pb_o = L.bo[w * 16 + c16], pg_1 = L.g1[w * 16 + c16], pe_1 = L.be1[w * 16 + c16];
    const float pb_2 = L.bo2[w * 16 + c16], pg_2 = L.g2[w * 16 + c16], pe_2 = L.be2[w * 16 + c16];
    h16x8<Hh> wq[4], wkv[2][4];
#pragma unroll
    for (int ks = 0; ks < 4; ++ks) {
      wq[ks] = gfrag(L.Wqkv, EH, w * 16, ks * 32, lane);
      wkv[0][ks] = gfrag(L.Wqkv, EH, EH + (2 * w) * 16, ks * 32, lane);
      wkv[1][ks] = gfrag(L.Wqkv, EH, EH + (2 * w + 1) * 16, ks * 32, lane);
    }
    if (l > 0) {
      if (tid == 0) {
        gu32_t* c = (gu32_t*)(cnt + (long long)samp * 6 + (l - 1));
        unsigned spins = 0;
        while (__hip_atomic_load(c, __ATOMIC_RELAXED, __HIP_MEMORY_SCOPE_AGENT) < (unsigned)NRT) {
          __builtin_amdgcn_s_sleep(4);
          if (++spins > RS_SPIN_MAX) { enc_give_up((gu32_t*)err); break; }
        }
      }
      __syncthreads();
    }
    RS_MARK(1);
    {
      const Hh* x = (l == 0 ? sg.x : sg.L[l - 1].out) + row_base * EH;
      const auto rsrc = __builtin_amdgcn_make_buffer_rsrc((void*)x, 0, N * EH * 2, 0x00020000);
      for (int id = tid; id < NRT * 16 * (EH / 8); id += NWAVE * 64) {
        const int r = id / (EH / 8), c = (id % (EH / 8)) * 8;
        const u32x4 v = __builtin_amdgcn_raw_buffer_load_b128(rsrc, (r * EH + c) * 2, 0, 16);
        *(u32x4*)(sX + r * XS + c) = v;
        if (r >= r0 && r < r0 + 16) *(u32x4*)(sO + (r - r0) * XS + c) = v;
      }
    }
    __syncthreads();
    RS_MARK(2);
    {
      f32x4 acc[NRT][2], aq = (f32x4){0.f, 0.f, 0.f, 0.f};
#pragma unroll
      for (int i = 0; i < NRT; ++i) { acc[i][0] = (f32x4){0.f, 0.f, 0.f, 0.f}; acc[i][1] = (f32x4){0.f, 0.f, 0.f, 0.f}; }
#pragma unroll
      for (int ks = 0; ks < 4; ++ks) {
#pragma unroll
        for (int i = 0; i < NRT; ++i) {
          const h16x8<Hh> a = frag_kc(sX, XS, i * 16, ks * 32, lane);
          acc[i][0] = mfma16(a, wkv[0][ks], acc[i][0]);
          acc[i][1] = mfma16(a, wkv[1][ks], acc[i][1]);
        }
        aq = mfma16(frag_kc(sO, XS, 0, ks * 32, lane), wq[ks], aq);
        KSTEP_FENCE();
      }
      Hh* dst = (w < 4 ? sK : sV) + ((2 * w) & 7) * 16 + c16;
#pragma unroll
      for (int i = 0; i < NRT; ++i)
#pragma unroll
        for (int r = 0; r < 4; ++r) {
          dst[(i * 16 + 4 * g + r) * XS] = from_f<Hh>(acc[i][0][r] + pb_kv0);
          dst[(i * 16 + 4 * g + r) * XS + 16] = from_f<Hh>(acc[i][1][r] + pb_kv1);
        }
#pragma unroll
      for (int r = 0; r < 4; ++r) sQ[(4 * g + r) * XS + w * 16 + c16] = from_f<Hh>(aq[r] + pb_q);
    }
    h16x8<Hh> wo[4], w1[4][4];
#pragma unroll
    for (int ks = 0; ks < 4; ++ks) wo[ks] = gfrag(L.Wo, EH, w * 16, ks * 32, lane);
#pragma unroll
    for (int ct = 0; ct < 4; ++ct)
#pragma unroll
      for (int ks = 0; ks < 4; ++ks) w1[ct][ks] = gfrag(L.W1, EH, (4 * w + ct) * 16, ks * 32, lane);
    __syncthreads();
    RS_MARK(3);
    {
      Hh* qg = L.qkv + row0 * 3 * EH;
      for (int id = tid; id < nq * 48; id += NWAVE * 64) {
        const int r = id / 48, c = (id % 48) * 8;
        const Hh* src = c < EH ? sQ + r * XS + c : (c < 2 * EH ? sK + (r0 + r) * XS + (c - EH) : sV + (r0 + r) * XS + (c - 2 * EH));
        *(h16x8<Hh>*)(qg + (long long)r * 3 * EH + c) = *(const h16x8<Hh>*)src;
      }
    }
    for (int u = w; u < ENH * NRT; u += NWAVE) {
      const int h = u / NRT, j = u % NRT;
      f32x4 sc = (f32x4){0.f, 0.f, 0.f, 0.f};
#pragma unroll
      for (int ks = 0; ks < 2; ++ks) sc = mfma16(frag_kc(sQ, XS, 0, h * EHD + ks * 32, lane), frag_kc(sK, XS, j * 16, h * EHD + ks * 32, lane), sc);
      const int key = j * 16 + c16;
      float mb = 0.f;
#pragma unroll
      for (int jj = 0; jj < NRT; ++jj) mb = (jj == j) ? kbias[jj] : mb;
#pragma unroll
      for (int r = 0; r < 4; ++r) sS[(h * 16 + 4 * g + r) * RS_SS + key] = key < N ? sc[r] * p.scale + mb : -3.0e38f;
    }
    __syncthreads();
    RS_MARK(4);
    dd.site = L.site_attn; dd.p = p.p_attn;
    const DropState dsa = drop_init(dd);
    {
      const int rr = 4 * w + g, h = rr >> 4, ql = rr & 15;
      float e[NRT], mx = -3.0e38f;
#pragma unroll
      for (int j = 0; j < NRT; ++j) { e[j] = sS[rr * RS_SS + j * 16 + c16]; mx = fmaxf(mx, e[j]); }
      mx = row16_max(mx);
      float sum = 0.f;
#pragma unroll
      for (int j = 0; j < NRT; ++j) { e[j] = (j * 16 + c16) < N ? __expf(e[j] - mx) : 0.f; sum += e[j]; }
      sum = 1.0f / row16_sum(sum);
      Hh* pc = (Hh*)(sS + rr * RS_SS);
      Hh* pd = sPd + rr * RS_PP;
#pragma unroll
      for (int j = 0; j < NRT; ++j) {
        const int key = j * 16 + c16;
        const float pv = e[j] * sum;
        pc[key] = from_f<Hh>(pv);
        if (dsa.on) {
          const unsigned idx = (unsigned)(((((long long)samp * ENH + h) * N + r0 + ql) * N) + key);
          pd[key] = from_f<Hh>((ql < nq && key < N) ? pv * drop_mul(dsa, idx) : 0.f);
        }
      }
      if (NRT * 16 < NKP && c16 < NKP - NRT * 16) { pc[NRT * 16 + c16] = (Hh)0.0f; if (dsa.on) pd[NRT * 16 + c16] = (Hh)0.0f; }
    }
    __syncthreads();
    RS_MARK(5);
    {
      const int cpr = ldp / 8;
      for (int id = tid; id < ENH * nq * cpr; id += NWAVE * 64) {
        const int h = id / (nq * cpr), rem = id % (nq * cpr), r = rem / cpr, c = (rem % cpr) * 8;
        const long long go = (((long long)samp * ENH + h) * N + r0 + r) * ldp + c;
        *(h16x8<Hh>*)(L.P + go) = *(const h16x8<Hh>*)((const Hh*)(sS + (h * 16 + r) * RS_SS) + c);
        if (dsa.on && L.Pd) *(h16x8<Hh>*)(L.Pd + go) = *(const h16x8<Hh>*)(sPd + (h * 16 + r) * RS_PP + c);
      }
    }
    {
      const int h = w >> 2, jd = w & 3;
      const Hh* pa = dsa.on ? sPd + h * 16 * RS_PP : (const Hh*)(sS + h * 16 * RS_SS);
      const int pp = dsa.on ? RS_PP : 2 * RS_SS;
      f32x4 o = (f32x4){0.f, 0.f, 0.f, 0.f};
      for (int ks = 0; ks < NKP / 32; ++ks)
        o = mfma16(frag_kc(pa, pp, 0, ks * 32, lane), tfrag_clamp(sV + h * EHD, XS, jd * 16, ks * 32, lane, NRT * 16), o);
#pragma unroll
      for (int r = 0; r < 4; ++r) sQ[(4 * g + r) * XS + h * EHD + jd * 16 + c16] = from_f<Hh>(o[r]);
    }
    __syncthreads();
    RS_MARK(6);
    copy_tile<false>(sQ, XS, L.ctx + row0 * EH, EH, nq, EH, tid);
    {
      f32x4 acc = (f32x4){0.f, 0.f, 0.f, 0.f};
#pragma unroll
      for (int ks = 0; ks < 4; ++ks) acc = mfma16(frag_kc(sQ, XS, 0, ks * 32, lane), wo[ks], acc);
      dd.site = L.site_ao; dd.p = p.p_hidden;
      const DropState dsh = drop_init(dd);
      add_norm16(acc, pb_o, pg_1, pe_1, sO, red, sA, L.rstd_a, nq, row0, p.eps, dsh, w, lane);
    }
    __syncthreads();
    RS_MARK(7);
    copy_tile<false>(sA, XS, L.a + row0 * EH, EH, nq, EH, tid);
    h16x8<Hh> w2[16];
    {
      f32x4 acc[4];
#pragma unroll
      for (int ct = 0; ct < 4; ++ct) acc[ct] = (f32x4){0.f, 0.f, 0.f, 0.f};
#pragma unroll
      for (int ks = 0; ks < 4; ++ks) {
        const h16x8<Hh> a = frag_kc(sA, XS, 0, ks * 32, lane);
#pragma unroll
        for (int ct = 0; ct < 4; ++ct) acc[ct] = mfma16(a, w1[ct][ks], acc[ct]);
      }
#pragma unroll
      for (int ks = 0; ks < 16; ++ks) w2[ks] = gfrag(L.W2, EI, w * 16, ks * 32, lane);
#pragma unroll
      for (int ct = 0; ct < 4; ++ct) {
        const int col = (4 * w + ct) * 16 + c16;
#pragma unroll
        for (int r = 0; r < 4; ++r) {
          const float zv = acc[ct][r] + pb_ffn[ct];
          sZ[(4 * g + r) * GS + col] = from_f<Hh>(zv);
          sG[(4 * g + r) * GS + col] = from_f<Hh>(gelu_fast(zv));
        }
      }
    }
    __syncthreads();
    RS_MARK(8);
    copy_tile<false>(sZ, GS, L.z + row0 * EI, EI, nq, EI, tid);
    copy_tile<false>(sG, GS, L.g + row0 * EI, EI, nq, EI, tid);
    {
      f32x4 acc = (f32x4){0.f, 0.f, 0.f, 0.f};
#pragma unroll
      for (int ks = 0; ks < 16; ++ks) acc = mfma16(frag_kc(sG, GS, 0, ks * 32, lane), w2[ks], acc);
      dd.site = L.site_out; dd.p = p.p_hidden;
      const DropState dsh = drop_init(dd);
      add_norm16(acc, pb_2, pg_2, pe_2, sA, red, sO, L.rstd_o, nq, row0, p.eps, dsh, w, lane);
    }
    __syncthreads();
    RS_MARK(9);
    copy_tile<true>(sO, XS, L.out + row0 * EH, EH, nq, EH, tid);
    asm volatile("s_waitcnt vmcnt(0)" ::: "memory");
    __syncthreads();
    RS_MARK(10);
    if (tid == 0 && l + 1 < sg.nlayers) __hip_atomic_fetch_add((gu32_t*)(cnt + (long long)samp * 6 + l), 1u, __ATOMIC_RELAXED, __HIP_MEMORY_SCOPE_AGENT);
  }
}

template <typename Hh>
__global__ __launch_bounds__(512) void encoder_rs_kernel(EncParamsT<Hh> p, int nt0, int nt1) {
  enc_mark_start();
  extern __shared__ __attribute__((aligned(16))) unsigned char enc_smem[];
  int b = blockIdx.x, s = 0, nt = nt0;
  unsigned* cnt = p.sync + 4;
  if (b >= p.seg[0].nsamp * nt0) { b -= p.seg[0].nsamp * nt0; s = 1; nt = nt1; cnt += 6ll * p.seg[0].nsamp; }
  const EncSegT<Hh>& sg = p.seg[s];
  const int samp = b / nt, tile = b - samp * nt;
  switch (nt) {
    case 1: enc_rs_body<1>(p, sg, samp, tile, cnt, p.sync, enc_smem); break;
    case 2: enc_rs_body<2>(p, sg, samp, tile, cnt, p.sync, enc_smem); break;
    case 3: enc_rs_body<3>(p, sg, samp, tile, cnt, p.sync, enc_smem); break;
    case 4: enc_rs_body<4>(p, sg, samp, tile, cnt, p.sync, enc_smem); break;
    default: enc_rs_body<5>(p, sg, samp, tile, cnt, p.sync, enc_smem); break;
  }
}
template <typename Hh>
__global__ __launch_bounds__(512) void encoder_mix_kernel(EncParamsT<Hh> p, int k0, int k1) {
  enc_mark_start();
  extern __shared__ __attribute__((aligned(16))) unsigned char enc_smem[];
  int b = blockIdx.x, s = 0, nt = k0;
  unsigned* cnt = p.sync + 4;
  const int blocks0 = p.seg[0].nsamp * k0;
  if (b >= blocks0) { b -= blocks0; s = 1; nt = k1; }
  const EncSegT<Hh>& sg = p.seg[s];
  const int na = nt > 0 ? nt : 1;
  const int samp = b / na, tile = b - samp * na;
  switch (nt) {
    case 4: enc_rs_body<4>(p, sg, samp, tile, cnt, p.sync, enc_smem); break;
    case 5: enc_rs_body<5>(p, sg, samp, tile, cnt, p.sync, enc_smem); break;
    case -3: enc_body<3>(p, sg, samp, enc_smem); break;
    default: enc_body<2>(p, sg, samp, enc_smem); break;
  }
}
static size_t enc_rs_lds_bytes() { return (size_t)(80 * XS + 81 * XS + 80 * XS + 3 * 16 * XS) * 2 + 256 * sizeof(float); }

static size_t enc_lds_bytes() {
  return (size_t)(2 * MAXROWS * XS + KROWS * QS + NWAVE * 16 * PSW) * 2 + (size_t)NWAVE * MAXROWS * sizeof(float);
}
static size_t enc_lds_bytes_compact() { return (size_t)(2 * 48 * XS + 49 * QS + 6 * 16 * 72) * 2; }

#define GATE_MAX_CONSEC 3
__global__ void enc_start_gate_kernel(long long timeout_ticks, long long recent_ticks, unsigned* st) {
  if (threadIdx.x) return;
  st[0] += 1;
  if (st[5]) {
    st[6] += 1;
    unsigned period = st[7] >> 16, n = (st[7] & 0xFFFFu) + 1;
    if (period == 0) period = 32;
    if (n >= period) { st[5] = 0; st[4] = 0; st[7] = (period < 1024 ? period * 2 : 1024) << 16; }
    else st[7] = (period << 16) | n;
    return;
  }
  const unsigned c0 = __hip_atomic_load(&magic_enc_starts, __ATOMIC_RELAXED, __HIP_MEMORY_SCOPE_AGENT);
  const long long t0 = wall_clock64();
  const long long tm = __hip_atomic_load(&magic_enc_start_tick, __ATOMIC_RELAXED, __HIP_MEMORY_SCOPE_AGENT);
  if (c0 != 0 && t0 - tm >= 0 && t0 - tm < recent_ticks) { st[2] += 1; st[4] = 0; st[7] = 0; return; }
  while (__hip_atomic_load(&magic_enc_starts, __ATOMIC_RELAXED, __HIP_MEMORY_SCOPE_AGENT) == c0) {
    if (wall_clock64() - t0 >= timeout_ticks) {
      st[3] += 1;
      if (++st[4] >= GATE_MAX_CONSEC) st[5] = 1;
      return;
    }
    __builtin_amdgcn_s_sleep(32);
  }
  st[1] += 1;
  st[4] = 0;
  st[7] = 0;
}
extern "C" int magic_encoder_start_gate(int timeout_us, int recent_us, unsigned* stats, void* stream) {
  if (timeout_us < 0 || timeout_us > 100000 || recent_us < 0 || recent_us > 100000 || !stats) return MAGIC_ERR_ARG;
  hipLaunchKernelGGL(enc_start_gate_kernel, dim3(1), dim3(64), 0, (hipStream_t)stream, (long long)timeout_us * 100, (long long)recent_us * 100, stats);
  return launch_status();
}

__global__ void stream_probe_wait_kernel(long long timeout_ticks, unsigned* w) {
  if (threadIdx.x) return;
  const long long t0 = wall_clock64();
  while (__hip_atomic_load(&w[0], __ATOMIC_RELAXED, __HIP_MEMORY_SCOPE_AGENT) == 0) {
    if (wall_clock64() - t0 >= timeout_ticks) { w[1] = 2; return; }
    __builtin_amdgcn_s_sleep(32);
  }
  w[1] = 1;
}
__global__ void stream_probe_set_kernel(unsigned* w) {
  if (threadIdx.x == 0) __hip_atomic_store(&w[0], 1u, __ATOMIC_RELAXED, __HIP_MEMORY_SCOPE_AGENT);
}
extern "C" int magic_stream_probe(unsigned* word2, int timeout_us, void* stream_wait, void* stream_set) {
  if (!word2 || timeout_us < 1 || timeout_us > 100000 || stream_wait == stream_set) return MAGIC_ERR_ARG;
  hipLaunchKernelGGL(stream_probe_wait_kernel, dim3(1), dim3(64), 0, (hipStream_t)stream_wait, (long long)timeout_us * 100, word2);
  if (int rc = launch_status()) return rc;
  hipLaunchKernelGGL(stream_probe_set_kernel, dim3(1), dim3(64), 0, (hipStream_t)stream_set, word2);
  return launch_status();
}

__global__ void enc_health_kernel(unsigned* out) {
  if (threadIdx.x == 0) {
    out[0] = __hip_atomic_load(&magic_enc_gave_up, __ATOMIC_RELAXED, __HIP_MEMORY_SCOPE_AGENT);
    out[1] = __hip_atomic_load(&magic_enc_starts, __ATOMIC_RELAXED, __HIP_MEMORY_SCOPE_AGENT);
  }
}
extern "C" int magic_encoder_health(unsigned* out, void* stream) {
  if (!out) return MAGIC_ERR_ARG;
  hipLaunchKernelGGL(enc_health_kernel, dim3(1), dim3(64), 0, (hipStream_t)stream, out);
  return launch_status();
}

extern "C" int magic_encoder_supported(int dtype, int H, int I, int nh, int N, int nlayers) {
  return dtype_is16(dtype) && H == EH && I == EI && nh == ENH && N >= 1 && N <= MAXROWS && nlayers >= 1 && nlayers <= 6;
}
extern "C" int magic_encoder_params_bytes() { return (int)sizeof(EncParams); }

extern "C" int magic_encoder_fwd(int dtype, const void* params, int nbytes, void* stream) {
  if (!params || nbytes != (int)sizeof(EncParams) || !dtype_is16(dtype)) return MAGIC_ERR_ARG;
  EncParams p;
  memcpy(&p, params, sizeof(p));
  if (p.nseg < 1 || p.nseg > 2) return MAGIC_ERR_ARG;
  if (!drop_args_ok(p.seed, p.p_attn) || !drop_args_ok(p.seed, p.p_hidden)) return MAGIC_ERR_ARG;
  int blocks = 0;
  for (int s = 0; s < 2; ++s) {
    EncSeg& sg = p.seg[s];
    if (s >= p.nseg) { sg.nsamp = 0; continue; }
    if (sg.nsamp <= 0 || sg.N < 1 || sg.N > MAXROWS || sg.nlayers < 1 || sg.nlayers > 6 || !sg.x) return MAGIC_ERR_ARG;
    if (sg.ldp < sg.N || (sg.ldp & 7) || sg.ldp > KROWS) return MAGIC_ERR_ARG;
    if ((long long)sg.nsamp * ENH * sg.N * sg.N > 0xFFFFFFFFll || (long long)sg.nsamp * sg.N * EI > 0x7FFFFFFFll) return MAGIC_ERR_ARG;
    if ((uintptr_t)sg.x & 15) return MAGIC_ERR_ARG;
    for (int l = 0; l < sg.nlayers; ++l) {
      const EncLayer& L = sg.L[l];
      const void* req[] = {L.Wqkv, L.bqkv, L.Wo, L.bo, L.g1, L.be1, L.W1, L.bi, L.W2, L.bo2, L.g2, L.be2, L.qkv, L.P, L.ctx, L.a, L.z, L.g, L.out, L.rstd_a, L.rstd_o};
      for (const void* q : req)
        if (!q) return MAGIC_ERR_ARG;
      const void* al[] = {L.Wqkv, L.Wo, L.W1, L.W2, L.qkv, L.P, L.Pd, L.ctx, L.a, L.g, L.out};
      for (const void* q : al)
        if ((uintptr_t)q & 15) return MAGIC_ERR_ARG;
      if (p.p_attn > 0.f && !L.Pd) return MAGIC_ERR_ARG;
    }
    blocks += sg.nsamp;
  }
  if (p.sync) {
    const int nt0 = (p.seg[0].N + 15) / 16, nt1 = p.nseg > 1 ? (p.seg[1].N + 15) / 16 : 1;
    const int ns1 = p.nseg > 1 ? p.seg[1].nsamp : 0;
    const long long words = 4 + 6ll * (p.seg[0].nsamp + ns1);
    if (p.sync_words < words || ((uintptr_t)p.sync & 15)) return MAGIC_ERR_ARG;
    static int ncu = 0;
    if (!ncu) { hipDeviceProp_t pr; int d = 0; (void)hipGetDevice(&d); ncu = (hipGetDeviceProperties(&pr, d) == hipSuccess) ? pr.multiProcessorCount : 256; }
    static int force = -2;
    if (force == -2) { const char* e = getenv("MAGIC_ENC_RS_ALL"); force = e ? atoi(e) : -1; }
    const bool rs0 = nt0 >= 4 && p.seg[0].nsamp * nt0 <= ncu, rs1 = p.nseg > 1 && nt1 >= 4 && p.seg[0].nsamp * nt0 + ns1 * nt1 <= ncu;
    const int form = (force == 1 || (rs0 && (rs1 || p.nseg == 1))) ? 2 : (rs0 && p.nseg == 2 && nt1 <= 3) ? 1 : 0;
    static bool rs_attr = false;
    if (!rs_attr) {
      (void)hipFuncSetAttribute((const void*)encoder_rs_kernel<bf16>, hipFuncAttributeMaxDynamicSharedMemorySize, (int)enc_rs_lds_bytes());
      (void)hipFuncSetAttribute((const void*)encoder_rs_kernel<f16>, hipFuncAttributeMaxDynamicSharedMemorySize, (int)enc_rs_lds_bytes());
      (void)hipFuncSetAttribute((const void*)encoder_mix_kernel<bf16>, hipFuncAttributeMaxDynamicSharedMemorySize, (int)enc_lds_bytes());
      (void)hipFuncSetAttribute((const void*)encoder_mix_kernel<f16>, hipFuncAttributeMaxDynamicSharedMemorySize, (int)enc_lds_bytes());
      rs_attr = true;
    }
    if (form) {
      if (hipMemsetAsync(p.sync, 0, (size_t)((words + 3) / 4 * 4) * sizeof(unsigned), (hipStream_t)stream) != hipSuccess) return MAGIC_ERR_LAUNCH;
      if (form == 2) {
        const int grid = p.seg[0].nsamp * nt0 + ns1 * nt1;
        DISPATCH_H(dtype, hipLaunchKernelGGL(encoder_rs_kernel<TY>, dim3(grid), dim3(512), enc_rs_lds_bytes(), (hipStream_t)stream, view_as<EncParamsT<TY>>(p), nt0, nt1));
      } else {
        const int grid = p.seg[0].nsamp * nt0 + ns1, k1 = -(nt1 < 2 ? 2 : nt1);
        const size_t shm_mix = enc_rs_lds_bytes() > enc_lds_bytes_compact() ? enc_rs_lds_bytes() : enc_lds_bytes_compact();
        DISPATCH_H(dtype, hipLaunchKernelGGL(encoder_mix_kernel<TY>, dim3(grid), dim3(512), shm_mix, (hipStream_t)stream, view_as<EncParamsT<TY>>(p), nt0, k1));
      }
      return launch_status();
    }
    if (hipMemsetAsync(p.sync, 0, 16, (hipStream_t)stream) != hipSuccess) return MAGIC_ERR_LAUNCH;
  }
  bool all_small = true;
  for (int sgi = 0; sgi < p.nseg; ++sgi) all_small = all_small && p.seg[sgi].N <= 48;
  const size_t shm = all_small ? enc_lds_bytes_compact() : enc_lds_bytes();
  static bool attr_set = false;
  if (!attr_set) {
    (void)hipFuncSetAttribute((const void*)encoder_fwd_kernel<bf16>, hipFuncAttributeMaxDynamicSharedMemorySize, (int)enc_lds_bytes());
    (void)hipFuncSetAttribute((const void*)encoder_fwd_kernel<f16>, hipFuncAttributeMaxDynamicSharedMemorySize, (int)enc_lds_bytes());
    attr_set = true;
  }
  DISPATCH_H(dtype, hipLaunchKernelGGL(encoder_fwd_kernel<TY>, dim3(blocks), dim3(512), shm, (hipStream_t)stream, view_as<EncParamsT<TY>>(p)));
  return launch_status();
}

template <typename Hh> struct XLayerT {
  const Hh* Wqkv; const float* bqkv; const Hh* Wo; const float* bo; const float* g1; const float* be1;
  const Hh* Wq; const float* bq; const Hh* Wkv; const float* bkv;
  const Hh* Woc; const float* boc; const float* gc; const float* bec;
  const Hh* W1; const float* bi; const Hh* W2; const float* bo2; const float* g2; const float* be2;
  Hh *qkv, *P, *Pd, *ctx, *a; float* rstd_a;
  Hh *q, *kv, *Pc, *Pdc, *cctx, *c; float* rstd_c;
  Hh *z, *g, *out; float* rstd_o;
  unsigned site_attn, site_ao, site_cattn, site_co, site_out, pad_;
};
template <typename Hh> struct XSegT {
  const Hh* x; const Hh* cx;
  const unsigned char* qmask; const unsigned char* cmask;
  const float* dist; const float* sprel_w; const float* sprel_b;
  int nsamp, Nq, Nk, ldps, ldpc, nlayers;
  XLayerT<Hh> L[3];
};
template <typename Hh> struct XParamsT {
  XSegT<Hh> seg[2]; int nseg; float p_attn, p_hidden, eps, scale; const unsigned* seed;
  unsigned* sync; int sync_words, pad2_;
};
typedef XParamsT<bf16> XParams; typedef XSegT<bf16> XSeg; typedef XLayerT<bf16> XLayer;
#define F(f) ABI_VIEW(XLayer, magic_xenc_layer, f)
F(Wqkv) F(bqkv) F(Wo) F(bo) F(g1) F(be1) F(Wq) F(bq) F(Wkv) F(bkv) F(Woc) F(boc) F(gc) F(bec) F(W1) F(bi) F(W2) F(bo2) F(g2) F(be2) F(qkv) F(P) F(Pd)
F(ctx) F(a) F(rstd_a) F(q) F(kv) F(Pc) F(Pdc) F(cctx) F(c) F(rstd_c) F(z) F(g) F(out) F(rstd_o) F(site_attn) F(site_ao) F(site_cattn) F(site_co)
F(site_out) F(pad_)
#undef F
#define F(f) ABI_VIEW(XSeg, magic_xenc_seg, f)
F(x) F(cx) F(qmask) F(cmask) F(dist) F(sprel_w) F(sprel_b) F(nsamp) F(Nq) F(Nk) F(ldps) F(ldpc) F(nlayers) F(L)
#undef F
#define F(f) ABI_VIEW(XParams, magic_xenc_params, f)
F(seg) F(nseg) F(p_attn) F(p_hidden) F(eps) F(scale) F(seed) F(sync) F(sync_words) F(pad2_)
#undef F

template <int NKT, typename Hh>
__device__ __forceinline__ void attn_unit(const Hh* sQKV, Hh* sPw, Hh* sCtx, Hh* Pg0, Hh* Pdg0, const int h, const int rt, const int Nq,
                                          const int Nk, const int ldp, const float (&kbias)[NKT], const float* dist, const float sw, const float sb,
                                          const long long samp, const float scale, const DropState& dsa, const int lane) {
  const int g = lane >> 4, c16 = lane & 15;
  const int NKP = (Nk + 31) / 32 * 32;
  f32x4 sc[NKT];
#pragma unroll
  for (int j = 0; j < NKT; ++j) sc[j] = (f32x4){0.f, 0.f, 0.f, 0.f};
#pragma unroll
  for (int ks = 0; ks < 2; ++ks) {
    const h16x8<Hh> a = frag_kc(sQKV, QS, rt * 16, h * EHD + ks * 32, lane);
#pragma unroll
    for (int j = 0; j < NKT; ++j) sc[j] = mfma16(a, frag_kc(sQKV, QS, j * 16, EH + h * EHD + ks * 32, lane), sc[j]);
  }
  float mx[4] = {-3.0e38f, -3.0e38f, -3.0e38f, -3.0e38f};
#pragma unroll
  for (int j = 0; j < NKT; ++j) {
    const int key = j * 16 + c16;
    const bool kv = key < Nk;
#pragma unroll
    for (int r = 0; r < 4; ++r) {
      float x = sc[j][r] * scale + kbias[j];
      if (dist && kv) { const int qrow = min(rt * 16 + 4 * g + r, Nq - 1); x += sw * dist[((long long)samp * Nq + qrow) * Nk + key] + sb; }
      x = kv ? x : -3.0e38f;
      sc[j][r] = x; mx[r] = fmaxf(mx[r], x);
    }
  }
  float sum[4];
#pragma unroll
  for (int r = 0; r < 4; ++r) { mx[r] = row16_max(mx[r]); sum[r] = 0.f; }
#pragma unroll
  for (int j = 0; j < NKT; ++j) {
    const bool kv = (j * 16 + c16) < Nk;
#pragma unroll
    for (int r = 0; r < 4; ++r) { const float e = kv ? __expf(sc[j][r] - mx[r]) : 0.f; sc[j][r] = e; sum[r] += e; }
  }
#pragma unroll
  for (int r = 0; r < 4; ++r) sum[r] = 1.0f / row16_sum(sum[r]);
#pragma unroll
  for (int j = 0; j < NKT; ++j)
#pragma unroll
    for (int r = 0; r < 4; ++r) sPw[(4 * g + r) * PSW + j * 16 + c16] = from_f<Hh>(sc[j][r] * sum[r]);
  if (NKT * 16 < NKP) {
    for (int id = lane; id < 16 * (NKP - NKT * 16); id += 64) {
      const int r = id / (NKP - NKT * 16), c = NKT * 16 + id % (NKP - NKT * 16);
      sPw[r * PSW + c] = (Hh)0.0f;
    }
  }
  wave_lds_sync();
  const int nq = min(16, Nq - rt * 16);
  {
    Hh* Pg = Pg0 + (((long long)samp * ENH + h) * Nq + rt * 16) * ldp;
    const int cpr = ldp / 8;
    for (int id = lane; id < nq * cpr; id += 64) {
      const int r = id / cpr, c = (id % cpr) * 8;
      *(h16x8<Hh>*)(Pg + (long long)r * ldp + c) = *(const h16x8<Hh>*)(sPw + r * PSW + c);
    }
  }
  if (dsa.on) {
#pragma unroll
    for (int j = 0; j < NKT; ++j) {
      const int key = j * 16 + c16;
#pragma unroll
      for (int r = 0; r < 4; ++r) {
        const int ql = 4 * g + r;
        const unsigned idx = (unsigned)(((((long long)samp * ENH + h) * Nq + rt * 16 + ql) * Nk) + key);
        const float m = (ql < nq && key < Nk) ? drop_mul(dsa, idx) : 0.f;
        sPw[ql * PSW + key] = from_f<Hh>(sc[j][r] * sum[r] * m);
      }
    }
    wave_lds_sync();
    if (Pdg0) {
      Hh* Pg = Pdg0 + (((long long)samp * ENH + h) * Nq + rt * 16) * ldp;
      const int cpr = ldp / 8;
      for (int id = lane; id < nq * cpr; id += 64) {
        const int r = id / cpr, c = (id % cpr) * 8;
        *(h16x8<Hh>*)(Pg + (long long)r * ldp + c) = *(const h16x8<Hh>*)(sPw + r * PSW + c);
      }
    }
  }
  f32x4 o[4];
#pragma unroll
  for (int jd = 0; jd < 4; ++jd) o[jd] = (f32x4){0.f, 0.f, 0.f, 0.f};
  for (int ks = 0; ks < NKP / 32; ++ks) {
    const h16x8<Hh> a = frag_kc(sPw, PSW, 0, ks * 32, lane);
#pragma unroll
    for (int jd = 0; jd < 4; ++jd) o[jd] = mfma16(a, frag_oc(sQKV + 2 * EH + h * EHD, QS, jd * 16, ks * 32, lane), o[jd]);
  }
#pragma unroll
  for (int jd = 0; jd < 4; ++jd)
#pragma unroll
    for (int r = 0; r < 4; ++r) sCtx[(rt * 16 + 4 * g + r) * XS + h * EHD + jd * 16 + c16] = from_f<Hh>(o[jd][r]);
}

template <int NRT, typename Hh>
__device__ __forceinline__ void proj16(f32x4 (&acc)[NRT], const Hh* sIn, const h16x8<Hh> (&wf)[4], const int lane) {
#pragma unroll
  for (int i = 0; i < NRT; ++i) acc[i] = (f32x4){0.f, 0.f, 0.f, 0.f};
#pragma unroll
  for (int ks = 0; ks < 4; ++ks) {
#pragma unroll
    for (int i = 0; i < NRT; ++i) acc[i] = mfma16(frag_kc(sIn, XS, i * 16, ks * 32, lane), wf[ks], acc[i]);
    KSTEP_FENCE();
  }
}

template <int NRT, typename Hh>
__device__ __forceinline__ void xenc_body(const XParamsT<Hh>& p, const XSegT<Hh>& sg, const int samp, unsigned char* smem) {
  constexpr int NKT = 5;
  Hh* sX = (Hh*)smem;
  Hh* sA = sX + MAXROWS * XS;
  Hh* sQKV = sA + MAXROWS * XS;
  Hh* sP = sQKV + KROWS * QS;
  Hh* sG = sQKV;
  float* red = (float*)(sP + NWAVE * 16 * PSW);
  const int tid = threadIdx.x, lane0 = tid & 63, w = __builtin_amdgcn_readfirstlane(tid >> 6);
  const int Nq = sg.Nq, Nk = sg.Nk;
  const long long qbase = (long long)samp * Nq, kbase = (long long)samp * Nk;
  constexpr int ROWS = NRT * 16;
  {
    const Hh* x = sg.x + qbase * EH;
    for (int id = tid; id < ROWS * (EH / 8); id += NWAVE * 64) {
      const int r = id / (EH / 8), c = (id % (EH / 8)) * 8;
      h16x8<Hh> v;
#pragma unroll
      for (int e = 0; e < 8; ++e) v[e] = (Hh)0.0f;
      if (r < Nq) v = *(const h16x8<Hh>*)(x + (long long)r * EH + c);
      *(h16x8<Hh>*)(sX + r * XS + c) = v;
    }
  }
  DropDesc dd;
  dd.seed = p.seed;
  float qbias[NRT], cbias[NKT];
#pragma unroll
  for (int j = 0; j < NRT; ++j) {
    const int key = j * 16 + (lane0 & 15);
    qbias[j] = (key < Nq && sg.qmask && !sg.qmask[qbase + key]) ? -10000.0f : 0.f;
  }
#pragma unroll
  for (int j = 0; j < NKT; ++j) {
    const int key = j * 16 + (lane0 & 15);
    cbias[j] = (key < Nk && sg.cmask && !sg.cmask[kbase + key]) ? -10000.0f : 0.f;
  }
  const float sw = sg.dist ? sg.sprel_w[0] : 0.f, sb = sg.dist ? sg.sprel_b[0] : 0.f;
  for (int l = 0; l < sg.nlayers; ++l) {
    const XLayerT<Hh>& L = sg.L[l];
    int lane = lane0;
    asm volatile("" : "+v"(lane));
    const int g = lane >> 4, c16 = lane & 15;
    const int colw = w * 16 + c16;
    float pb_qkv[3], pb_ffn[4], pb_kv[2];
#pragma unroll
    for (int ct = 0; ct < 3; ++ct) pb_qkv[ct] = L.bqkv[(3 * w + ct) * 16 + c16];
#pragma unroll
    for (int ct = 0; ct < 4; ++ct) pb_ffn[ct] = L.bi[(4 * w + ct) * 16 + c16];
#pragma unroll
    for (int ct = 0; ct < 2; ++ct) pb_kv[ct] = L.bkv[(2 * w + ct) * 16 + c16];
    const float pb_o = L.bo[colw], pg_1 = L.g1[colw], pe_1 = L.be1[colw], pb_q = L.bq[colw];
    const float pb_oc = L.boc[colw], pg_c = L.gc[colw], pe_c = L.bec[colw];
    const float pb_2 = L.bo2[colw], pg_2 = L.g2[colw], pe_2 = L.be2[colw];
    h16x8<Hh> bw[3][4];
#pragma unroll
    for (int ct = 0; ct < 3; ++ct)
#pragma unroll
      for (int ks = 0; ks < 4; ++ks) bw[ct][ks] = gfrag(L.Wqkv, EH, (3 * w + ct) * 16, ks * 32, lane);
    for (int id = tid; id < (KROWS - ROWS) * (384 / 8); id += NWAVE * 64) {
      const int r = ROWS + id / 48, c = (id % 48) * 8;
      h16x8<Hh> zv;
#pragma unroll
      for (int e = 0; e < 8; ++e) zv[e] = (Hh)0.0f;
      *(h16x8<Hh>*)(sQKV + r * QS + c) = zv;
    }
    __syncthreads();
    {
      f32x4 acc[NRT][3];
#pragma unroll
      for (int i = 0; i < NRT; ++i)
#pragma unroll
        for (int ct = 0; ct < 3; ++ct) acc[i][ct] = (f32x4){0.f, 0.f, 0.f, 0.f};
#pragma unroll
      for (int ks = 0; ks < 4; ++ks) {
#pragma unroll
        for (int i = 0; i < NRT; ++i) {
          const h16x8<Hh> a = frag_kc(sX, XS, i * 16, ks * 32, lane);
#pragma unroll
          for (int ct = 0; ct < 3; ++ct) acc[i][ct] = mfma16(a, bw[ct][ks], acc[i][ct]);
        }
        KSTEP_FENCE();
      }
#pragma unroll
      for (int ct = 0; ct < 3; ++ct) {
        const int col = (3 * w + ct) * 16 + c16;
#pragma unroll
        for (int i = 0; i < NRT; ++i)
#pragma unroll
          for (int r = 0; r < 4; ++r) sQKV[(i * 16 + 4 * g + r) * QS + col] = from_f<Hh>(acc[i][ct][r] + pb_qkv[ct]);
      }
    }
    h16x8<Hh> wo[4], wq[4];
#pragma unroll
    for (int ks = 0; ks < 4; ++ks) { wo[ks] = gfrag(L.Wo, EH, w * 16, ks * 32, lane); wq[ks] = gfrag(L.Wq, EH, w * 16, ks * 32, lane); }
    __syncthreads();
    copy_out(sQKV, QS, L.qkv + qbase * 3 * EH, 3 * EH, Nq, 3 * EH, tid);
    dd.site = L.site_attn; dd.p = p.p_attn;
    const DropState dsa = drop_init(dd);
    Hh* sPw = sP + w * 16 * PSW;
    for (int u = w; u < ENH * NRT; u += NWAVE)
      attn_unit<NRT>(sQKV, sPw, sA, L.P, L.Pd, u / NRT, u % NRT, Nq, Nq, sg.ldps, qbias, sg.dist, sw, sb, samp, p.scale, dsa, lane);
    __syncthreads();
    copy_out(sA, XS, L.ctx + qbase * EH, EH, Nq, EH, tid);
    {
      f32x4 acc[NRT];
      proj16<NRT>(acc, sA, wo, lane);
      dd.site = L.site_ao; dd.p = p.p_hidden;
      const DropState dsh = drop_init(dd);
      add_norm<NRT, MAXROWS>(acc, pb_o, pg_1, pe_1, sX, red, sA, L.rstd_a, Nq, qbase, p.eps, dsh, w, lane);
    }
    h16x8<Hh> wkv[2][4];
#pragma unroll
    for (int ct = 0; ct < 2; ++ct)
#pragma unroll
      for (int ks = 0; ks < 4; ++ks) wkv[ct][ks] = gfrag(L.Wkv, EH, (2 * w + ct) * 16, ks * 32, lane);
    __syncthreads();
    copy_out(sA, XS, L.a + qbase * EH, EH, Nq, EH, tid);
    {
      f32x4 acc[NRT];
      proj16<NRT>(acc, sA, wq, lane);
#pragma unroll
      for (int i = 0; i < NRT; ++i)
#pragma unroll
        for (int r = 0; r < 4; ++r) sQKV[(i * 16 + 4 * g + r) * QS + colw] = from_f<Hh>(acc[i][r] + pb_q);
    }
    {
      f32x4 acc[NKT][2];
#pragma unroll
      for (int i = 0; i < NKT; ++i)
#pragma unroll
        for (int ct = 0; ct < 2; ++ct) acc[i][ct] = (f32x4){0.f, 0.f, 0.f, 0.f};
      const Hh* cx = sg.cx + kbase * EH;
#pragma unroll
      for (int ks = 0; ks < 4; ++ks) {
#pragma unroll
        for (int i = 0; i < NKT; ++i) {
          const int row = min(i * 16 + c16, Nk - 1);
          const h16x8<Hh> a = *(const h16x8<Hh>*)(cx + (long long)row * EH + ks * 32 + 8 * g);
#pragma unroll
          for (int ct = 0; ct < 2; ++ct) acc[i][ct] = mfma16(a, wkv[ct][ks], acc[i][ct]);
        }
        KSTEP_FENCE();
      }
#pragma unroll
      for (int ct = 0; ct < 2; ++ct) {
        const int col = EH + (2 * w + ct) * 16 + c16;
#pragma unroll
        for (int i = 0; i < NKT; ++i)
#pragma unroll
          for (int r = 0; r < 4; ++r) {
            const int row = i * 16 + 4 * g + r;
            sQKV[row * QS + col] = (row < Nk) ? from_f<Hh>(acc[i][ct][r] + pb_kv[ct]) : (Hh)0.0f;
          }
      }
    }
    for (int id = tid; id < (KROWS - NKT * 16) * (256 / 8); id += NWAVE * 64) {
      const int r = NKT * 16 + id / 32, c = EH + (id % 32) * 8;
      h16x8<Hh> zv;
#pragma unroll
      for (int e = 0; e < 8; ++e) zv[e] = (Hh)0.0f;
      *(h16x8<Hh>*)(sQKV + r * QS + c) = zv;
    }
    h16x8<Hh> woc[4];
#pragma unroll
    for (int ks = 0; ks < 4; ++ks) woc[ks] = gfrag(L.Woc, EH, w * 16, ks * 32, lane);
    h16x8<Hh> w1[4][4];
#pragma unroll
    for (int ct = 0; ct < 4; ++ct)
#pragma unroll
      for (int ks = 0; ks < 4; ++ks) w1[ct][ks] = gfrag(L.W1, EH, (4 * w + ct) * 16, ks * 32, lane);
    __syncthreads();
    copy_out(sQKV, QS, L.q + qbase * EH, EH, Nq, EH, tid);
    copy_out(sQKV + EH, QS, L.kv + kbase * 2 * EH, 2 * EH, Nk, 2 * EH, tid);
    dd.site = L.site_cattn; dd.p = p.p_attn;
    const DropState dsc = drop_init(dd);
    for (int u = w; u < ENH * NRT; u += NWAVE)
      attn_unit<NKT>(sQKV, sPw, sX, L.Pc, L.Pdc, u / NRT, u % NRT, Nq, Nk, sg.ldpc, cbias, nullptr, 0.f, 0.f, samp, p.scale, dsc, lane);
    __syncthreads();
    copy_out(sX, XS, L.cctx + qbase * EH, EH, Nq, EH, tid);
    {
      f32x4 acc[NRT];
      proj16<NRT>(acc, sX, woc, lane);
      dd.site = L.site_co; dd.p = p.p_hidden;
      const DropState dsh = drop_init(dd);
      add_norm<NRT, MAXROWS>(acc, pb_oc, pg_c, pe_c, sA, red, sX, L.rstd_c, Nq, qbase, p.eps, dsh, w, lane);
    }
    __syncthreads();
    copy_out(sX, XS, L.c + qbase * EH, EH, Nq, EH, tid);
    h16x8<Hh> w2[16];
    {
      f32x4 acc[NRT][4];
#pragma unroll
      for (int i = 0; i < NRT; ++i)
#pragma unroll
        for (int ct = 0; ct < 4; ++ct) acc[i][ct] = (f32x4){0.f, 0.f, 0.f, 0.f};
#pragma unroll
      for (int ks = 0; ks < 4; ++ks) {
#pragma unroll
        for (int i = 0; i < NRT; ++i) {
          const h16x8<Hh> a = frag_kc(sX, XS, i * 16, ks * 32, lane);
#pragma unroll
          for (int ct = 0; ct < 4; ++ct) acc[i][ct] = mfma16(a, w1[ct][ks], acc[i][ct]);
        }
        KSTEP_FENCE();
      }
#pragma unroll
      for (int ks = 0; ks < 16; ++ks) w2[ks] = gfrag(L.W2, EI, w * 16, ks * 32, lane);
#pragma unroll
      for (int ct = 0; ct < 4; ++ct) {
        const int col = (4 * w + ct) * 16 + c16;
#pragma unroll
        for (int i = 0; i < NRT; ++i)
#pragma unroll
          for (int r = 0; r < 4; ++r) {
            acc[i][ct][r] += pb_ffn[ct];
            sG[(i * 16 + 4 * g + r) * GS + col] = from_f<Hh>(acc[i][ct][r]);
          }
      }
      __syncthreads();
      copy_out(sG, GS, L.z + qbase * EI, EI, Nq, EI, tid);
#pragma unroll
      for (int ct = 0; ct < 4; ++ct)
#pragma unroll
        for (int i = 0; i < NRT; ++i)
#pragma unroll
          for (int r = 0; r < 4; ++r) acc[i][ct][r] = gelu_fast(acc[i][ct][r]);
      __syncthreads();
#pragma unroll
      for (int ct = 0; ct < 4; ++ct) {
        const int col = (4 * w + ct) * 16 + c16;
#pragma unroll
        for (int i = 0; i < NRT; ++i)
#pragma unroll
          for (int r = 0; r < 4; ++r) sG[(i * 16 + 4 * g + r) * GS + col] = from_f<Hh>(acc[i][ct][r]);
      }
    }
    __syncthreads();
    copy_out(sG, GS, L.g + qbase * EI, EI, Nq, EI, tid);
    {
      f32x4 acc[NRT];
#pragma unroll
      for (int i = 0; i < NRT; ++i) acc[i] = (f32x4){0.f, 0.f, 0.f, 0.f};
#pragma unroll
      for (int ks = 0; ks < 16; ++ks) {
#pragma unroll
        for (int i = 0; i < NRT; ++i) acc[i] = mfma16(frag_kc(sG, GS, i * 16, ks * 32, lane), w2[ks], acc[i]);
        if ((ks & 1) == 1) KSTEP_FENCE();
      }
      dd.site = L.site_out; dd.p = p.p_hidden;
      const DropState dsh = drop_init(dd);
      add_norm<NRT, MAXROWS>(acc, pb_2, pg_2, pe_2, sX, red, sX, L.rstd_o, Nq, qbase, p.eps, dsh, w, lane);
    }
    __syncthreads();
    copy_out(sX, XS, L.out + qbase * EH, EH, Nq, EH, tid);
  }
}

template <int NKT, typename Hh>
__device__ __forceinline__ void rs_attn(Hh* sQ, const Hh* sK, const Hh* sV, float* sS, Hh* sPd, const float (&kbias)[NKT], const int Nk, const int kmax,
                                        const float* dist, const float sw, const float sb, const int q0, const int nq, const int Nq,
                                        Hh* Pg, Hh* Pdg, const int ldp, const long long samp, const float scale, const DropState& dsa,
                                        const int tid, const int w, const int lane) {
  const int g = lane >> 4, c16 = lane & 15;
  const int NKP = (Nk + 31) / 32 * 32;
  for (int u = w; u < ENH * NKT; u += NWAVE) {
    const int h = u / NKT, j = u % NKT;
    f32x4 sc = (f32x4){0.f, 0.f, 0.f, 0.f};
#pragma unroll
    for (int ks = 0; ks < 2; ++ks) sc = mfma16(frag_kc(sQ, XS, 0, h * EHD + ks * 32, lane), frag_kc(sK, XS, j * 16, h * EHD + ks * 32, lane), sc);
    const int key = j * 16 + c16;
    float mb = 0.f;
#pragma unroll
    for (int jj = 0; jj < NKT; ++jj) mb = (jj == j) ? kbias[jj] : mb;
#pragma unroll
    for (int r = 0; r < 4; ++r) {
      float x = sc[r] * scale + mb;
      if (dist && key < Nk) { const int qrow = min(q0 + 4 * g + r, Nq - 1); x += sw * dist[((long long)samp * Nq + qrow) * Nk + key] + sb; }
      sS[(h * 16 + 4 * g + r) * RS_SS + key] = key < Nk ? x : -3.0e38f;
    }
  }
  __syncthreads();
  {
    const int rr = 4 * w + g, h = rr >> 4, ql = rr & 15;
    float e[NKT], mx = -3.0e38f;
#pragma unroll
    for (int j = 0; j < NKT; ++j) { e[j] = sS[rr * RS_SS + j * 16 + c16]; mx = fmaxf(mx, e[j]); }
    mx = row16_max(mx);
    float sum = 0.f;
#pragma unroll
    for (int j = 0; j < NKT; ++j) { e[j] = (j * 16 + c16) < Nk ? __expf(e[j] - mx) : 0.f; sum += e[j]; }
    sum = 1.0f / row16_sum(sum);
    Hh* pc = (Hh*)(sS + rr * RS_SS);
    Hh* pd = sPd + rr * RS_PP;
#pragma unroll
    for (int j = 0; j < NKT; ++j) {
      const int key = j * 16 + c16;
      const float pv = e[j] * sum;
      pc[key] = from_f<Hh>(pv);
      if (dsa.on) {
        const unsigned idx = (unsigned)(((((long long)samp * ENH + h) * Nq + q0 + ql) * Nk) + key);
        pd[key] = from_f<Hh>((ql < nq && key < Nk) ? pv * drop_mul(dsa, idx) : 0.f);
      }
    }
    if (NKT * 16 < NKP && c16 < NKP - NKT * 16) { pc[NKT * 16 + c16] = (Hh)0.0f; if (dsa.on) pd[NKT * 16 + c16] = (Hh)0.0f; }
  }
  __syncthreads();
  {
    const int cpr = ldp / 8;
    for (int id = tid; id < ENH * nq * cpr; id += NWAVE * 64) {
      const int h = id / (nq * cpr), rem = id % (nq * cpr), r = rem / cpr, c = (rem % cpr) * 8;
      const long long go = (((long long)samp * ENH + h) * Nq + q0 + r) * ldp + c;
      *(h16x8<Hh>*)(Pg + go) = *(const h16x8<Hh>*)((const Hh*)(sS + (h * 16 + r) * RS_SS) + c);
      if (dsa.on && Pdg) *(h16x8<Hh>*)(Pdg + go) = *(const h16x8<Hh>*)(sPd + (h * 16 + r) * RS_PP + c);
    }
  }
  {
    const int h = w >> 2, jd = w & 3;
    const Hh* pa = dsa.on ? sPd + h * 16 * RS_PP : (const Hh*)(sS + h * 16 * RS_SS);
    const int pp = dsa.on ? RS_PP : 2 * RS_SS;
    f32x4 o = (f32x4){0.f, 0.f, 0.f, 0.f};
    for (int ks = 0; ks < NKP / 32; ++ks)
      o = mfma16(frag_kc(pa, pp, 0, ks * 32, lane), tfrag_clamp(sV + h * EHD, XS, jd * 16, ks * 32, lane, kmax), o);
#pragma unroll
    for (int r = 0; r < 4; ++r) sQ[(4 * g + r) * XS + h * EHD + jd * 16 + c16] = from_f<Hh>(o[r]);
  }
  __syncthreads();
}

template <int NRT, typename Hh>
__device__ __forceinline__ void xenc_rs_body(const XParamsT<Hh>& p, const XSegT<Hh>& sg, const int samp, const int tile, const int ntile,
                                             unsigned* cnt, unsigned* err, unsigned char* smem) {
  constexpr int NKT = 5;
  Hh* sK = (Hh*)smem;
  Hh* sV = sK + 80 * XS;
  Hh* sU = sV + 81 * XS;
  Hh* sX = sU;
  float* sS = (float*)sU;
  Hh* sPd = sU + 2 * 16 * RS_SS * 2;
  Hh* sG = sU;
  Hh* sZ = sK;
  Hh* sQ = sU + 80 * XS;
  Hh* sO = sQ + 16 * XS;
  Hh* sA = sO + 16 * XS;
  float* red = (float*)(sA + 16 * XS);
  const int tid = threadIdx.x, lane0 = tid & 63, w = __builtin_amdgcn_readfirstlane(tid >> 6);
  const int Nq = sg.Nq, Nk = sg.Nk;
  const long long qbase = (long long)samp * Nq, kbase = (long long)samp * Nk;
  const int r0 = tile * 16, nq = min(16, Nq - r0);
  const long long row0 = qbase + r0;
  if (tid < XS / 8) {
    h16x8<Hh> zv;
#pragma unroll
    for (int e = 0; e < 8; ++e) zv[e] = (Hh)0.0f;
    *(h16x8<Hh>*)(sV + RS_ZROW * XS + tid * 8) = zv;
  }
  DropDesc dd;
  dd.seed = p.seed;
  float qbias[NRT], cbias[NKT];
#pragma unroll
  for (int j = 0; j < NRT; ++j) {
    const int key = j * 16 + (lane0 & 15);
    qbias[j] = (key < Nq && sg.qmask && !sg.qmask[qbase + key]) ? -10000.0f : 0.f;
  }
#pragma unroll
  for (int j = 0; j < NKT; ++j) {
    const int key = j * 16 + (lane0 & 15);
    cbias[j] = (key < Nk && sg.cmask && !sg.cmask[kbase + key]) ? -10000.0f : 0.f;
  }
  const float sw = sg.dist ? sg.sprel_w[0] : 0.f, sb = sg.dist ? sg.sprel_b[0] : 0.f;
  for (int l = 0; l < sg.nlayers; ++l) {
    const XLayerT<Hh>& L = sg.L[l];
    int lane = lane0;
    asm volatile("" : "+v"(lane));
    const int g = lane >> 4, c16 = lane & 15;
    const int colw = w * 16 + c16;
    const float pb_q0 = L.bqkv[colw], pb_kv0 = L.bqkv[EH + (2 * w) * 16 + c16], pb_kv1 = L.bqkv[EH + (2 * w + 1) * 16 + c16];
    const float pb_ck0 = L.bkv[(2 * w) * 16 + c16], pb_ck1 = L.bkv[(2 * w + 1) * 16 + c16];
    float pb_ffn[4];
#pragma unroll
    for (int ct = 0; ct < 4; ++ct) pb_ffn[ct] = L.bi[(4 * w + ct) * 16 + c16];
    const float pb_o = L.bo[colw], pg_1 = L.g1[colw], pe_1 = L.be1[colw], pb_q = L.bq[colw];
    const float pb_oc = L.boc[colw], pg_c = L.gc[colw], pe_c = L.bec[colw];
    const float pb_2 = L.bo2[colw], pg_2 = L.g2[colw], pe_2 = L.be2[colw];
    h16x8<Hh> wq[4], wkv[2][4];
#pragma unroll
    for (int ks = 0; ks < 4; ++ks) {
      wq[ks] = gfrag(L.Wqkv, EH, w * 16, ks * 32, lane);
      wkv[0][ks] = gfrag(L.Wqkv, EH, EH + (2 * w) * 16, ks * 32, lane);
      wkv[1][ks] = gfrag(L.Wqkv, EH, EH + (2 * w + 1) * 16, ks * 32, lane);
    }
    if (l > 0) {
      if (tid == 0) {
        gu32_t* c = (gu32_t*)(cnt + (long long)samp * 6 + (l - 1));
        unsigned spins = 0;
        while (__hip_atomic_load(c, __ATOMIC_RELAXED, __HIP_MEMORY_SCOPE_AGENT) < (unsigned)ntile) {
          __builtin_amdgcn_s_sleep(4);
          if (++spins > RS_SPIN_MAX) { enc_give_up((gu32_t*)err); break; }
        }
      }
      __syncthreads();
    }
    {
      const Hh* x = (l == 0 ? sg.x : sg.L[l - 1].out) + qbase * EH;
      const auto rsrc = __builtin_amdgcn_make_buffer_rsrc((void*)x, 0, Nq * EH * 2, 0x00020000);
      for (int id = tid; id < NRT * 16 * (EH / 8); id += NWAVE * 64) {
        const int r = id / (EH / 8), c = (id % (EH / 8)) * 8;
        const u32x4 v = __builtin_amdgcn_raw_buffer_load_b128(rsrc, (r * EH + c) * 2, 0, 16);
        *(u32x4*)(sX + r * XS + c) = v;
        if (r >= r0 && r < r0 + 16) *(u32x4*)(sO + (r - r0) * XS + c) = v;
      }
    }
    __syncthreads();
    {
      f32x4 acc[NRT][2], aq = (f32x4){0.f, 0.f, 0.f, 0.f};
#pragma unroll
      for (int i = 0; i < NRT; ++i) { acc[i][0] = (f32x4){0.f, 0.f, 0.f, 0.f}; acc[i][1] = (f32x4){0.f, 0.f, 0.f, 0.f}; }
#pragma unroll
      for (int ks = 0; ks < 4; ++ks) {
#pragma unroll
        for (int i = 0; i < NRT; ++i) {
          const h16x8<Hh> a = frag_kc(sX, XS, i * 16, ks * 32, lane);
          acc[i][0] = mfma16(a, wkv[0][ks], acc[i][0]);
          acc[i][1] = mfma16(a, wkv[1][ks], acc[i][1]);
        }
        aq = mfma16(frag_kc(sO, XS, 0, ks * 32, lane), wq[ks], aq);
        KSTEP_FENCE();
      }
      Hh* dst = (w < 4 ? sK : sV) + ((2 * w) & 7) * 16 + c16;
#pragma unroll
      for (int i = 0; i < NRT; ++i)
#pragma unroll
        for (int r = 0; r < 4; ++r) {
          dst[(i * 16 + 4 * g + r) * XS] = from_f<Hh>(acc[i][0][r] + pb_kv0);
          dst[(i * 16 + 4 * g + r) * XS + 16] = from_f<Hh>(acc[i][1][r] + pb_kv1);
        }
#pragma unroll
      for (int r = 0; r < 4; ++r) sQ[(4 * g + r) * XS + colw] = from_f<Hh>(aq[r] + pb_q0);
    }
    h16x8<Hh> wo[4], wcq[4];
#pragma unroll
    for (int ks = 0; ks < 4; ++ks) { wo[ks] = gfrag(L.Wo, EH, w * 16, ks * 32, lane); wcq[ks] = gfrag(L.Wq, EH, w * 16, ks * 32, lane); }
    __syncthreads();
    {
      Hh* qg = L.qkv + row0 * 3 * EH;
      for (int id = tid; id < nq * 48; id += NWAVE * 64) {
        const int r = id / 48, c = (id % 48) * 8;
        const Hh* src = c < EH ? sQ + r * XS + c : (c < 2 * EH ? sK + (r0 + r) * XS + (c - EH) : sV + (r0 + r) * XS + (c - 2 * EH));
        *(h16x8<Hh>*)(qg + (long long)r * 3 * EH + c) = *(const h16x8<Hh>*)src;
      }
    }
    dd.site = L.site_attn; dd.p = p.p_attn;
    const DropState dsa = drop_init(dd);
    rs_attn<NRT>(sQ, sK, sV, sS, sPd, qbias, Nq, NRT * 16, sg.dist, sw, sb, r0, nq, Nq, L.P, L.Pd, sg.ldps, samp, p.scale, dsa, tid, w, lane);
    copy_tile<false>(sQ, XS, L.ctx + row0 * EH, EH, nq, EH, tid);
    {
      f32x4 acc = (f32x4){0.f, 0.f, 0.f, 0.f};
#pragma unroll
      for (int ks = 0; ks < 4; ++ks) acc = mfma16(frag_kc(sQ, XS, 0, ks * 32, lane), wo[ks], acc);
      dd.site = L.site_ao; dd.p = p.p_hidden;
      const DropState dsh = drop_init(dd);
      add_norm16(acc, pb_o, pg_1, pe_1, sO, red, sA, L.rstd_a, nq, row0, p.eps, dsh, w, lane);
    }
    h16x8<Hh> wck[2][4];
#pragma unroll
    for (int ct = 0; ct < 2; ++ct)
#pragma unroll
      for (int ks = 0; ks < 4; ++ks) wck[ct][ks] = gfrag(L.Wkv, EH, (2 * w + ct) * 16, ks * 32, lane);
    __syncthreads();
    copy_tile<false>(sA, XS, L.a + row0 * EH, EH, nq, EH, tid);
    {
      f32x4 aq = (f32x4){0.f, 0.f, 0.f, 0.f};
#pragma unroll
      for (int ks = 0; ks < 4; ++ks) aq = mfma16(frag_kc(sA, XS, 0, ks * 32, lane), wcq[ks], aq);
#pragma unroll
      for (int r = 0; r < 4; ++r) sQ[(4 * g + r) * XS + colw] = from_f<Hh>(aq[r] + pb_q);
      f32x4 acc[NKT][2];
#pragma unroll
      for (int i = 0; i < NKT; ++i) { acc[i][0] = (f32x4){0.f, 0.f, 0.f, 0.f}; acc[i][1] = (f32x4){0.f, 0.f, 0.f, 0.f}; }
      const Hh* cx = sg.cx + kbase * EH;
#pragma unroll
      for (int ks = 0; ks < 4; ++ks) {
#pragma unroll
        for (int i = 0; i < NKT; ++i) {
          const int row = min(i * 16 + c16, Nk - 1);
          const h16x8<Hh> a = *(const h16x8<Hh>*)(cx + (long long)row * EH + ks * 32 + 8 * g);
          acc[i][0] = mfma16(a, wck[0][ks], acc[i][0]);
          acc[i][1] = mfma16(a, wck[1][ks], acc[i][1]);
        }
        KSTEP_FENCE();
      }
      Hh* dst = (w < 4 ? sK : sV) + ((2 * w) & 7) * 16 + c16;
#pragma unroll
      for (int i = 0; i < NKT; ++i)
#pragma unroll
        for (int r = 0; r < 4; ++r) {
          const int row = i * 16 + 4 * g + r;
          dst[row * XS] = row < Nk ? from_f<Hh>(acc[i][0][r] + pb_ck0) : (Hh)0.0f;
          dst[row * XS + 16] = row < Nk ? from_f<Hh>(acc[i][1][r] + pb_ck1) : (Hh)0.0f;
        }
    }
    h16x8<Hh> woc[4], w1[4][4];
#pragma unroll
    for (int ks = 0; ks < 4; ++ks) woc[ks] = gfrag(L.Woc, EH, w * 16, ks * 32, lane);
#pragma unroll
    for (int ct = 0; ct < 4; ++ct)
#pragma unroll
      for (int ks = 0; ks < 4; ++ks) w1[ct][ks] = gfrag(L.W1, EH, (4 * w + ct) * 16, ks * 32, lane);
    __syncthreads();
    copy_tile<false>(sQ, XS, L.q + row0 * EH, EH, nq, EH, tid);
    for (int kt = tile; kt * 16 < Nk; kt += ntile) {
      const int nr = min(16, Nk - kt * 16);
      Hh* kg = L.kv + (kbase + kt * 16) * 2 * EH;
      for (int id = tid; id < nr * 32; id += NWAVE * 64) {
        const int r = id / 32, c = (id % 32) * 8;
        const Hh* src = c < EH ? sK + (kt * 16 + r) * XS + c : sV + (kt * 16 + r) * XS + (c - EH);
        *(h16x8<Hh>*)(kg + (long long)r * 2 * EH + c) = *(const h16x8<Hh>*)src;
      }
    }
    dd.site = L.site_cattn; dd.p = p.p_attn;
    const DropState dsc = drop_init(dd);
    rs_attn<NKT>(sQ, sK, sV, sS, sPd, cbias, Nk, NKT * 16, nullptr, 0.f, 0.f, r0, nq, Nq, L.Pc, L.Pdc, sg.ldpc, samp, p.scale, dsc, tid, w, lane);
    copy_tile<false>(sQ, XS, L.cctx + row0 * EH, EH, nq, EH, tid);
    {
      f32x4 acc = (f32x4){0.f, 0.f, 0.f, 0.f};
#pragma unroll
      for (int ks = 0; ks < 4; ++ks) acc = mfma16(frag_kc(sQ, XS, 0, ks * 32, lane), woc[ks], acc);
      dd.site = L.site_co; dd.p = p.p_hidden;
      const DropState dsh = drop_init(dd);
      add_norm16(acc, pb_oc, pg_c, pe_c, sA, red, sO, L.rstd_c, nq, row0, p.eps, dsh, w, lane);
    }
    __syncthreads();
    copy_tile<false>(sO, XS, L.c + row0 * EH, EH, nq, EH, tid);
    h16x8<Hh> w2[16];
    {
      f32x4 acc[4];
#pragma unroll
      for (int ct = 0; ct < 4; ++ct) acc[ct] = (f32x4){0.f, 0.f, 0.f, 0.f};
#pragma unroll
      for (int ks = 0; ks < 4; ++ks) {
        const h16x8<Hh> a = frag_kc(sO, XS, 0, ks * 32, lane);
#pragma unroll
        for (int ct = 0; ct < 4; ++ct) acc[ct] = mfma16(a, w1[ct][ks], acc[ct]);
      }
#pragma unroll
      for (int ks = 0; ks < 16; ++ks) w2[ks] = gfrag(L.W2, EI, w * 16, ks * 32, lane);
#pragma unroll
      for (int ct = 0; ct < 4; ++ct) {
        const int col = (4 * w + ct) * 16 + c16;
#pragma unroll
        for (int r = 0; r < 4; ++r) {
          const float zv = acc[ct][r] + pb_ffn[ct];
          sZ[(4 * g + r) * GS + col] = from_f<Hh>(zv);
          sG[(4 * g + r) * GS + col] = from_f<Hh>(gelu_fast(zv));
        }
      }
    }
    __syncthreads();
    copy_tile<false>(sZ, GS, L.z + row0 * EI, EI, nq, EI, tid);
    copy_tile<false>(sG, GS, L.g + row0 * EI, EI, nq, EI, tid);
    {
      f32x4 acc = (f32x4){0.f, 0.f, 0.f, 0.f};
#pragma unroll
      for (int ks = 0; ks < 16; ++ks) acc = mfma16(frag_kc(sG, GS, 0, ks * 32, lane), w2[ks], acc);
      dd.site = L.site_out; dd.p = p.p_hidden;
      const DropState dsh = drop_init(dd);
      add_norm16(acc, pb_2, pg_2, pe_2, sO, red, sA, L.rstd_o, nq, row0, p.eps, dsh, w, lane);
    }
    __syncthreads();
    copy_tile<true>(sA, XS, L.out + row0 * EH, EH, nq, EH, tid);
    asm volatile("s_waitcnt vmcnt(0)" ::: "memory");
    __syncthreads();
    if (tid == 0 && l + 1 < sg.nlayers) __hip_atomic_fetch_add((gu32_t*)(cnt + (long long)samp * 6 + l), 1u, __ATOMIC_RELAXED, __HIP_MEMORY_SCOPE_AGENT);
  }
}

template <typename Hh>
__global__ __launch_bounds__(512) void xencoder_rs_kernel(XParamsT<Hh> p, int nt0, int nt1) {
  extern __shared__ __attribute__((aligned(16))) unsigned char enc_smem[];
  int b = blockIdx.x, s = 0, nt = nt0;
  unsigned* cnt = p.sync + 4;
  if (b >= p.seg[0].nsamp * nt0) { b -= p.seg[0].nsamp * nt0; s = 1; nt = nt1; cnt += 6ll * p.seg[0].nsamp; }
  const XSegT<Hh>& sg = p.seg[s];
  const int samp = b / nt, tile = b - samp * nt;
  if (nt <= 3) xenc_rs_body<3>(p, sg, samp, tile, nt, cnt, p.sync, enc_smem);
  else xenc_rs_body<5>(p, sg, samp, tile, nt, cnt, p.sync, enc_smem);
}

template <typename Hh>
__global__ __launch_bounds__(512) void xencoder_fwd_kernel(XParamsT<Hh> p) {
  extern __shared__ __attribute__((aligned(16))) unsigned char enc_smem[];
  int b = blockIdx.x, s = 0;
  if (b >= p.seg[0].nsamp) { b -= p.seg[0].nsamp; s = 1; }
  const XSegT<Hh>& sg = p.seg[s];
  const int nrt = max(2, (sg.Nq + 15) / 16);
  switch (nrt) {
    case 2: xenc_body<2>(p, sg, b, enc_smem); break;
    case 3: xenc_body<3>(p, sg, b, enc_smem); break;
    case 4: xenc_body<4>(p, sg, b, enc_smem); break;
    default: xenc_body<5>(p, sg, b, enc_smem); break;
  }
}

extern "C" int magic_xencoder_supported(int dtype, int H, int I, int nh, int Nq, int Nk, int nlayers) {
  return dtype_is16(dtype) && H == EH && I == EI && nh == ENH && Nq >= 1 && Nq <= MAXROWS && Nk >= 1 && Nk <= MAXROWS && nlayers >= 1 && nlayers <= 3;
}
extern "C" int magic_xencoder_params_bytes() { return (int)sizeof(XParams); }

extern "C" int magic_xencoder_fwd(int dtype, const void* params, int nbytes, void* stream) {
  if (!params || nbytes != (int)sizeof(XParams) || !dtype_is16(dtype)) return MAGIC_ERR_ARG;
  XParams p;
  memcpy(&p, params, sizeof(p));
  if (p.nseg < 1 || p.nseg > 2) return MAGIC_ERR_ARG;
  if (!drop_args_ok(p.seed, p.p_attn) || !drop_args_ok(p.seed, p.p_hidden)) return MAGIC_ERR_ARG;
  int blocks = 0;
  for (int s = 0; s < 2; ++s) {
    XSeg& sg = p.seg[s];
    if (s >= p.nseg) { sg.nsamp = 0; continue; }
    if (sg.nsamp <= 0 || sg.Nq < 1 || sg.Nq > MAXROWS || sg.Nk < 1 || sg.Nk > MAXROWS || sg.nlayers < 1 || sg.nlayers > 3 || !sg.x || !sg.cx) return MAGIC_ERR_ARG;
    if (sg.ldps < sg.Nq || (sg.ldps & 7) || sg.ldps > KROWS || sg.ldpc < sg.Nk || (sg.ldpc & 7) || sg.ldpc > KROWS) return MAGIC_ERR_ARG;
    if ((long long)sg.nsamp * ENH * sg.Nq * MAXROWS > 0xFFFFFFFFll) return MAGIC_ERR_ARG;
    if (((uintptr_t)sg.x & 15) || ((uintptr_t)sg.cx & 15)) return MAGIC_ERR_ARG;
    if (sg.dist && (!sg.sprel_w || !sg.sprel_b)) return MAGIC_ERR_ARG;
    for (int l = 0; l < sg.nlayers; ++l) {
      const XLayer& L = sg.L[l];
      const void* req[] = {L.Wqkv, L.bqkv, L.Wo, L.bo, L.g1, L.be1, L.Wq, L.bq, L.Wkv, L.bkv, L.Woc, L.boc, L.gc, L.bec, L.W1, L.bi, L.W2, L.bo2, L.g2, L.be2,
                           L.qkv, L.P, L.ctx, L.a, L.rstd_a, L.q, L.kv, L.Pc, L.cctx, L.c, L.rstd_c, L.z, L.g, L.out, L.rstd_o};
      for (const void* q : req)
        if (!q) return MAGIC_ERR_ARG;
      const void* al[] = {L.Wqkv, L.Wo, L.Wq, L.Wkv, L.Woc, L.W1, L.W2, L.qkv, L.P, L.Pd, L.ctx, L.a, L.q, L.kv, L.Pc, L.Pdc, L.cctx, L.c, L.z, L.g, L.out};
      for (const void* q : al)
        if ((uintptr_t)q & 15) return MAGIC_ERR_ARG;
      if (p.p_attn > 0.f && (!L.Pd || !L.Pdc)) return MAGIC_ERR_ARG;
    }
    blocks += sg.nsamp;
  }
  if (p.sync) {
    const int nt0 = (p.seg[0].Nq + 15) / 16, nt1 = p.nseg > 1 ? (p.seg[1].Nq + 15) / 16 : 1;
    const int ns1 = p.nseg > 1 ? p.seg[1].nsamp : 0;
    const long long words = 4 + 6ll * (p.seg[0].nsamp + ns1);
    if (p.sync_words < words || ((uintptr_t)p.sync & 15)) return MAGIC_ERR_ARG;
    static int ncu = 0;
    if (!ncu) { hipDeviceProp_t pr; int d = 0; (void)hipGetDevice(&d); ncu = (hipGetDeviceProperties(&pr, d) == hipSuccess) ? pr.multiProcessorCount : 256; }
    const int grid = p.seg[0].nsamp * nt0 + ns1 * nt1;
    if (grid <= ncu && grid > blocks) {
      static bool rs_attr = false;
      if (!rs_attr) {
        (void)hipFuncSetAttribute((const void*)xencoder_rs_kernel<bf16>, hipFuncAttributeMaxDynamicSharedMemorySize, (int)enc_rs_lds_bytes());
        (void)hipFuncSetAttribute((const void*)xencoder_rs_kernel<f16>, hipFuncAttributeMaxDynamicSharedMemorySize, (int)enc_rs_lds_bytes());
        rs_attr = true;
      }
      if (hipMemsetAsync(p.sync, 0, (size_t)((words + 3) / 4 * 4) * sizeof(unsigned), (hipStream_t)stream) != hipSuccess) return MAGIC_ERR_LAUNCH;
      DISPATCH_H(dtype, hipLaunchKernelGGL(xencoder_rs_kernel<TY>, dim3(grid), dim3(512), enc_rs_lds_bytes(), (hipStream_t)stream, view_as<XParamsT<TY>>(p), nt0, nt1));
      return launch_status();
    }
    if (hipMemsetAsync(p.sync, 0, 16, (hipStream_t)stream) != hipSuccess) return MAGIC_ERR_LAUNCH;
  }
  const size_t shm = enc_lds_bytes();
  static bool attr_set = false;
  if (!attr_set) {
    (void)hipFuncSetAttribute((const void*)xencoder_fwd_kernel<bf16>, hipFuncAttributeMaxDynamicSharedMemorySize, (int)shm);
    (void)hipFuncSetAttribute((const void*)xencoder_fwd_kernel<f16>, hipFuncAttributeMaxDynamicSharedMemorySize, (int)shm);
    attr_set = true;
  }
  DISPATCH_H(dtype, hipLaunchKernelGGL(xencoder_fwd_kernel<TY>, dim3(blocks), dim3(512), shm, (hipStream_t)stream, view_as<XParamsT<TY>>(p)));
  return launch_status();
}
```

Measured before the change: 200,600.

## Stage row loads through registers and prefetch context fragments across encoder kernels

```diff
diff --git a/profiles/micro/chain_timing.hip b/profiles/micro/chain_timing.hip
--- a/profiles/micro/chain_timing.hip
+++ b/profiles/micro/chain_timing.hip
@@ -6,7 +6,7 @@
   const int M = argc > 1 ? atoi(argv[1]) : 3840;
   ChainParams P; memset(&P, 0, sizeof(P));
   P.M = M; P.ld_in = CH; P.Np = 3 * CH; P.eps = 1e-12f;
-  P.in = dmalloc((size_t)M * CH * 2, 0x11); P.res = dmalloc((size_t)M * CH * 2, 0x11);
+  P.inp = dmalloc((size_t)M * CH * 2, 0x11); P.res = dmalloc((size_t)M * CH * 2, 0x11);
   P.Wa = dmalloc(CH * CH * 2, 0x11); P.ba = (float*)dmalloc(CH * 4, 0); P.g1 = (float*)dmalloc(CH * 4, 0x3c); P.b1 = (float*)dmalloc(CH * 4, 0);
   P.W1 = dmalloc(CI * CH * 2, 0x11); P.bi = (float*)dmalloc(CI * 4, 0); P.W2 = dmalloc(CI * CH * 2, 0x11); P.bo2 = (float*)dmalloc(CH * 4, 0);
   P.g2 = (float*)dmalloc(CH * 4, 0x3c); P.b2 = (float*)dmalloc(CH * 4, 0); P.y2 = dmalloc((size_t)M * CH * 2, 0);
diff --git a/profiles/micro/enc_stage_loads_bits.py b/profiles/micro/enc_stage_loads_bits.py
--- /dev/null
+++ b/profiles/micro/enc_stage_loads_bits.py
@@ -0,0 +1,90 @@
+import argparse
+import hashlib
+import os
+import subprocess
+import sys
+
+ROOT = os.path.dirname(os.path.dirname(os.path.dirname(os.path.abspath(__file__))))
+sys.path.insert(0, ROOT)
+
+
+def digest(t):
+    import torch
+    return hashlib.sha256(t.detach().contiguous().cpu().reshape(-1).view(torch.uint8).numpy().tobytes()).hexdigest()[:16]
+
+
+def child(path):
+    import torch
+    from tests import test_encoder_fp64_gpu as E
+    from tests import test_enc_stage_loads_gpu as T
+    out = {}
+
+    def take(tag, segs):
+        torch.cuda.synchronize()
+        for k, v in T.outputs_of(segs):
+            out[f"{tag} {k}"] = digest(v)
+
+    for dt in ("bf16", "fp16"):
+        for p in (0.0, 0.1):
+            for case in T.ENC:
+                segs, seed = T.build_enc(case, dt, p)
+                E.launch_enc(segs, p, seed)
+                take(f"enc {case[0]} {dt} p={p}", segs)
+            sg, seed = T.build_full49(dt, p)
+            T.launch_without_sync(sg, p, seed)
+            take(f"enc full49-nosync {dt} p={p}", [sg])
+            for case in T.XENC:
+                for nl in (1, 3):
+                    sg, seed = T.build_xenc(case, dt, nl, p)
+                    E.launch_xenc([sg], p, seed)
+                    take(f"xenc {case[0]} x{nl} {dt} p={p}", [sg])
+        for kind in T.KINDS:
+            for n, _ in T.HOLES:
+                sg, seed = T.build_holes(n, kind, dt)
+                E.launch_enc([sg], 0.1, seed)
+                take(f"holes {kind} N={n} {dt}", [sg])
+            for nq, nk, _ in T.XHOLES:
+                sg, seed = T.build_xholes(nq, nk, kind, dt)
+                E.launch_xenc([sg], 0.1, seed)
+                take(f"xholes {kind} {nq}x{nk} {dt}", [sg])
+    for dtype, dn in ((torch.bfloat16, "bf16"), (torch.float16, "fp16")):
+        for rows, M in T.CHAIN:
+            for ffn, n_proj, store_y1 in T.CHAIN_FORMS:
+                _, _, _, outs = T.run_chain(rows, M, ffn, n_proj, store_y1, dtype)
+                for k, pair in outs.items():
+                    if pair is not None:
+                        out[f"chain rows{rows} M={M} ffn={int(ffn)} {dn} {k}"] = digest(pair[1])
+    with open(path, "w") as fh:
+        for k in sorted(out):
+            fh.write(f"{out[k]} {k}\n")
+
+
+def main():
+    ap = argparse.ArgumentParser()
+    ap.add_argument("--other", help="the library to compare this tree's build with")
+    ap.add_argument("--out", default=None)
+    ap.add_argument("--child", default=None)
+    a = ap.parse_args()
+    if a.child:
+        return child(a.child)
+    tmp = os.path.join(ROOT, "profile_out")
+    os.makedirs(tmp, exist_ok=True)
+    res = {}
+    for tag, env in (("this", {}), ("other", {"MAGIC_LIB_FILE": os.path.abspath(a.other), "MAGIC_ALLOW_STALE_LIB": "1"})):
+        path = os.path.join(tmp, f"enc_stage_loads_bits_{tag}.txt")
+        subprocess.run([sys.executable, os.path.abspath(__file__), "--child", path], check=True, env={**os.environ, **env}, cwd=ROOT, timeout=600)
+        res[tag] = dict(line.rstrip("\n").split(" ", 1)[::-1] for line in open(path))
+    keys = sorted(set(res["this"]) | set(res["other"]))
+    diff = [k for k in keys if res["this"].get(k) != res["other"].get(k)]
+    lines = [f"enc_stage_loads_bits: {len(keys)} output tensors of {len({k.rsplit(' ', 1)[0] for k in keys})} cases compared between this tree's library and the other build",
+             f"differing tensors: {len(diff)}"] + [f"  DIFFERS {k}" for k in diff]
+    text = "\n".join(lines) + "\n"
+    sys.stdout.write(text)
+    if a.out:
+        with open(a.out, "w") as fh:
+            fh.write(text)
+    return 1 if diff else 0
+
+
+if __name__ == "__main__":
+    sys.exit(main())
diff --git a/profiles/micro/enc_stage_loads_probe.hip b/profiles/micro/enc_stage_loads_probe.hip
--- /dev/null
+++ b/profiles/micro/enc_stage_loads_probe.hip
@@ -0,0 +1,101 @@
+#include "../../vln-magic_amd/csrc/encoder.hip"
+#include <algorithm>
+#include <cstdio>
+#include <vector>
+static void* dmalloc(size_t n, int fill) { void* p; hipMalloc(&p, n); hipMemset(p, fill, n); return p; }
+static long long med(std::vector<long long> v) { std::sort(v.begin(), v.end()); return v[v.size() / 2]; }
+#define BF(n, fill) (bf16*)dmalloc((size_t)(n) * 2, fill)
+#define FL(n, fill) (float*)dmalloc((size_t)(n) * 4, fill)
+int main() {
+  const int B = 48, L = 80, Np = 290, V = 36, REP = 20;
+  unsigned* seed = (unsigned*)dmalloc(8, 0x5a);
+  EncParams P; memset(&P, 0, sizeof(P));
+  P.nseg = 2; P.eps = 1e-12f; P.scale = 0.125f; P.seed = seed; P.p_attn = 0.1f; P.p_hidden = 0.1f;
+  auto fill_seg = [&](EncSeg& s, int ns, int N, int nl) {
+    s.nsamp = ns; s.N = N; s.ldp = (N + 7) / 8 * 8; s.nlayers = nl;
+    const size_t M = (size_t)ns * N;
+    s.x = BF(M * EH, 0x11); s.kmask = (const unsigned char*)dmalloc(M, 1);
+    for (int l = 0; l < nl; ++l) {
+      EncLayer& E = s.L[l];
+      E.Wqkv = BF(3 * EH * EH, 0x11); E.bqkv = FL(3 * EH, 0); E.Wo = BF(EH * EH, 0x11); E.bo = FL(EH, 0); E.g1 = FL(EH, 0x3c); E.be1 = FL(EH, 0);
+      E.W1 = BF(EI * EH, 0x11); E.bi = FL(EI, 0); E.W2 = BF(EH * EI, 0x11); E.bo2 = FL(EH, 0); E.g2 = FL(EH, 0x3c); E.be2 = FL(EH, 0);
+      E.qkv = BF(M * 3 * EH, 0); E.P = BF((size_t)ns * ENH * N * s.ldp, 0); E.Pd = BF((size_t)ns * ENH * N * s.ldp, 0);
+      E.ctx = BF(M * EH, 0); E.a = BF(M * EH, 0); E.z = BF(M * EI, 0); E.g = BF(M * EI, 0); E.out = BF(M * EH, 0);
+      E.rstd_a = FL(M, 0); E.rstd_o = FL(M, 0);
+      E.site_attn = 11 + l; E.site_ao = 21 + l; E.site_out = 31 + l;
+    }
+  };
+  fill_seg(P.seg[0], B, L, 6);
+  fill_seg(P.seg[1], Np, V, 2);
+  P.sync_words = 4 + 6 * (B + Np) + 4; P.sync = (unsigned*)dmalloc(P.sync_words * 4, 0);
+  {
+    std::vector<long long> entry, pano, reload[6];
+    long long t[8][16], e[2][16];
+    for (int it = 0; it < 3 + REP; ++it) {
+      if (magic_encoder_fwd(DT_BF16, &P, sizeof(P), nullptr) != 0) { printf("magic_encoder_fwd failed\n"); return 1; }
+      if (hipDeviceSynchronize() != hipSuccess) { printf("encoder launch faulted\n"); return 1; }
+      if (it < 3) continue;
+      hipMemcpyFromSymbol(t, HIP_SYMBOL(rs_ticks), sizeof(t)); hipMemcpyFromSymbol(e, HIP_SYMBOL(enc_ticks), sizeof(e));
+      entry.push_back(t[0][2] - t[0][11]); pano.push_back(e[1][10] - e[1][9]);
+      for (int l = 0; l < 6; ++l) reload[l].push_back(t[l][2] - t[l][1]);
+    }
+    unsigned err; hipMemcpy(&err, P.sync, 4, hipMemcpyDeviceToHost);
+    printf("encoder_mix text 48x80x6 + pano 290x36x2, dropout 0.1, give-up word %u; medians of %d launches, 10 ns ticks\n", err, REP);
+    printf("  text tile 0: entry -> first barrier %lld; reload l=0..5:", med(entry));
+    for (int l = 0; l < 6; ++l) printf(" %lld", med(reload[l]));
+    printf("\n  pano sample 0: prologue (mask bytes + layer-0 rows) %lld\n", med(pano));
+  }
+  XParams X; memset(&X, 0, sizeof(X));
+  X.nseg = 2; X.eps = 1e-12f; X.scale = 0.125f; X.seed = seed; X.p_attn = 0.1f; X.p_hidden = 0.1f;
+  auto fill_x = [&](XSeg& s, int ns, int Nq, int Nk, bool dist) {
+    s.nsamp = ns; s.Nq = Nq; s.Nk = Nk; s.ldps = (Nq + 7) / 8 * 8; s.ldpc = (Nk + 7) / 8 * 8; s.nlayers = 3;
+    const size_t M = (size_t)ns * Nq, Mk = (size_t)ns * Nk;
+    s.x = BF(M * EH, 0x11); s.cx = BF(Mk * EH, 0x11);
+    s.qmask = (const unsigned char*)dmalloc(M, 1); s.cmask = (const unsigned char*)dmalloc(Mk, 1);
+    if (dist) { s.dist = FL((size_t)ns * Nq * Nq, 0); s.sprel_w = FL(1, 0); s.sprel_b = FL(1, 0); }
+    for (int l = 0; l < 3; ++l) {
+      XLayer& E = s.L[l];
+      E.Wqkv = BF(3 * EH * EH, 0x11); E.bqkv = FL(3 * EH, 0); E.Wo = BF(EH * EH, 0x11); E.bo = FL(EH, 0); E.g1 = FL(EH, 0x3c); E.be1 = FL(EH, 0);
+      E.Wq = BF(EH * EH, 0x11); E.bq = FL(EH, 0); E.Wkv = BF(2 * EH * EH, 0x11); E.bkv = FL(2 * EH, 0); E.Woc = BF(EH * EH, 0x11); E.boc = FL(EH, 0);
+      E.gc = FL(EH, 0x3c); E.bec = FL(EH, 0);
+      E.W1 = BF(EI * EH, 0x11); E.bi = FL(EI, 0); E.W2 = BF(EH * EI, 0x11); E.bo2 = FL(EH, 0); E.g2 = FL(EH, 0x3c); E.be2 = FL(EH, 0);
+      E.qkv = BF(M * 3 * EH, 0); E.P = BF((size_t)ns * ENH * Nq * s.ldps, 0); E.Pd = BF((size_t)ns * ENH * Nq * s.ldps, 0);
+      E.ctx = BF(M * EH, 0); E.a = BF(M * EH, 0); E.rstd_a = FL(M, 0);
+      E.q = BF(M * EH, 0); E.kv = BF(Mk * 2 * EH, 0); E.Pc = BF((size_t)ns * ENH * Nq * s.ldpc, 0); E.Pdc = BF((size_t)ns * ENH * Nq * s.ldpc, 0);
+      E.cctx = BF(M * EH, 0); E.c = BF(M * EH, 0); E.rstd_c = FL(M, 0);
+      E.z = BF(M * EI, 0); E.g = BF(M * EI, 0); E.out = BF(M * EH, 0); E.rstd_o = FL(M, 0);
+      E.site_attn = 41 + l; E.site_ao = 51 + l; E.site_cattn = 61 + l; E.site_co = 71 + l; E.site_out = 81 + l;
+    }
+  };
+  fill_x(X.seg[0], B, 37, 80, true);
+  fill_x(X.seg[1], B, 20, 80, false);
+  X.sync_words = 4 + 6 * (2 * B) + 4; X.sync = (unsigned*)dmalloc(X.sync_words * 4, 0);
+  {
+    std::vector<long long> entry, reload[3], ckv[3], total;
+    long long t[8][16];
+    for (int it = 0; it < 3 + REP; ++it) {
+      if (magic_xencoder_fwd(DT_BF16, &X, sizeof(X), nullptr) != 0) { printf("magic_xencoder_fwd failed\n"); return 1; }
+      if (hipDeviceSynchronize() != hipSuccess) { printf("cross encoder launch faulted\n"); return 1; }
+      if (it < 3) continue;
+      hipMemcpyFromSymbol(t, HIP_SYMBOL(xrs_ticks), sizeof(t));
+      entry.push_back(t[0][2] - t[0][11]);
+      for (int l = 0; l < 3; ++l) { reload[l].push_back(t[l][2] - t[l][1]); ckv[l].push_back(t[l][4] - t[l][3]); }
+      total.push_back(t[2][4] - t[0][11]);
+    }
+    unsigned err; hipMemcpy(&err, X.sync, 4, hipMemcpyDeviceToHost);
+    printf("xencoder_rs 48 x (37 | 20) queries x 80 context rows x 3 layers, dropout 0.1, give-up word %u; medians of %d launches, 10 ns ticks\n", err, REP);
+    printf("  tile 0: entry -> first barrier %lld; reload l=0..2: %lld %lld %lld; ctx K|V l=0..2: %lld %lld %lld; entry -> last ctx K|V barrier %lld\n",
+           med(entry), med(reload[0]), med(reload[1]), med(reload[2]), med(ckv[0]), med(ckv[1]), med(ckv[2]), med(total));
+  }
+  hipEvent_t e0, e1; hipEventCreate(&e0); hipEventCreate(&e1);
+  float ms;
+  hipEventRecord(e0);
+  for (int it = 0; it < REP; ++it) magic_encoder_fwd(DT_BF16, &P, sizeof(P), nullptr);
+  hipEventRecord(e1); hipEventSynchronize(e1); hipEventElapsedTime(&ms, e0, e1);
+  printf("encoder_mix launch (memset + kernel): %.1f us\n", ms * 1000 / REP);
+  hipEventRecord(e0);
+  for (int it = 0; it < REP; ++it) magic_xencoder_fwd(DT_BF16, &X, sizeof(X), nullptr);
+  hipEventRecord(e1); hipEventSynchronize(e1); hipEventElapsedTime(&ms, e0, e1);
+  printf("xencoder_rs launch (memset + kernel): %.1f us\n", ms * 1000 / REP);
+  return 0;
+}
diff --git a/vln-magic_amd/csrc/chain.hip b/vln-magic_amd/csrc/chain.hip
--- a/vln-magic_amd/csrc/chain.hip
+++ b/vln-magic_amd/csrc/chain.hip
@@ -79,14 +79,22 @@
     }
 }
 
-template <typename Hh>
-__device__ __forceinline__ void chain_rows_in(const Hh* src, long long ld, int nq, Hh* dst, int tid) {
-  typedef __attribute__((ext_vector_type(4))) unsigned u4;
-  for (int id = tid; id < CROWS * (CH / 8); id += NWAVE * 64) {
-    const int r = id / (CH / 8), c = (id % (CH / 8)) * 8;
-    const u4 v = r < nq ? *(const u4*)(src + r * ld + c) : (u4){0u, 0u, 0u, 0u};
-    *(u4*)(dst + CADDR(r, c, KP)) = v;
-  }
+template <int ROWS, typename Hh> struct ChainRows {
+  static constexpr int NIT = ROWS * (CH / 8) / (NWAVE * 64);
+  RowImg<Hh> iIn, iRes;
+  rowvec<Hh> rIn[NIT], rRes[NIT];
+};
+template <int ROWS, typename Hh>
+__device__ __forceinline__ void chain_rows_issue(ChainRows<ROWS, Hh>& cr, const ChainParams& p, int row0, int nq, Hh* sIn, Hh* sRes, int pitch, int tid) {
+  cr.iIn = RowImg<Hh>{sIn, pitch, (const Hh*)p.inp + (long long)row0 * p.ld_in, p.ld_in, nq, CH, CH / 8, ROWS * (CH / 8)};
+  cr.iRes = RowImg<Hh>{sRes, pitch, (const Hh*)p.res + (long long)row0 * CH, CH, nq, CH, CH / 8, ROWS * (CH / 8)};
+  stage_issue<ChainRows<ROWS, Hh>::NIT>(cr.rIn, cr.iIn, 0, tid, NWAVE * 64);
+  stage_issue<ChainRows<ROWS, Hh>::NIT>(cr.rRes, cr.iRes, 0, tid, NWAVE * 64);
+}
+template <int ROWS, typename Hh>
+__device__ __forceinline__ void chain_rows_store(const ChainRows<ROWS, Hh>& cr, int tid) {
+  stage_store<ChainRows<ROWS, Hh>::NIT>(cr.rIn, cr.iIn, 0, tid, NWAVE * 64);
+  stage_store<ChainRows<ROWS, Hh>::NIT>(cr.rRes, cr.iRes, 0, tid, NWAVE * 64);
 }
 
 template <typename Hh> __device__ __forceinline__ h16x8<Hh> pfrag(const Hh* __restrict__ Wf, const int K, const int nt, const int ks, const int lane) {
@@ -140,14 +148,15 @@
 #define SEQ(s) (FFN ? (s) : ((s) < 2 ? (s) : (s) + 16))
 #define AHEAD(s) do { if ((s) + CNB - 1 < NS) chain_load_chunk<Hh>(ring[((s) + CNB - 1) % CNB], SEQ((s) + CNB - 1), p, w, lane, nct); } while (0)
   CH_MARK(0);
-  chain_rows_in((const Hh*)p.inp + (long long)row0 * p.ld_in, p.ld_in, nq, sIn, tid);
-  chain_rows_in((const Hh*)p.res + (long long)row0 * CH, CH, nq, sRes, tid);
+  ChainRows<CROWS, Hh> rows;
+  chain_rows_issue(rows, p, row0, nq, sIn, sRes, KP, tid);
   if (tid < CH) {
     sPar[tid] = p.ba[tid]; sPar[CH + tid] = p.g1[tid]; sPar[2 * CH + tid] = p.b1[tid];
     if (FFN) { sPar[3 * CH + tid] = p.bo2[tid]; sPar[4 * CH + tid] = p.g2[tid]; sPar[5 * CH + tid] = p.b2[tid]; }
   }
   if (FFN) { sPar[6 * CH + tid] = p.bi[tid]; sPar[6 * CH + 512 + tid] = p.bi[512 + tid]; }
   for (int i = tid; i < nct * 128; i += NWAVE * 64) sPar[6 * CH + CI + i] = p.bp[i];
+  chain_rows_store(rows, tid);
   h16x8<Hh> ring[CNB][8];
 #pragma unroll
   for (int s = 0; s < CNB - 1; ++s) chain_load_chunk<Hh>(ring[s], SEQ(s), p, w, lane, nct);
@@ -362,15 +371,6 @@
         sOut[row * CP + col] = from_f<Hh>(acc[rt][i] * r4[r] * gv + btv);
       }
     }
-}
-template <typename Hh>
-__device__ __forceinline__ void chain64_rows_in(const Hh* src, long long ld, int nq, Hh* dst, int tid) {
-  typedef __attribute__((ext_vector_type(4))) unsigned u4;
-  for (int id = tid; id < C6ROWS * (CH / 8); id += NWAVE * 64) {
-    const int r = id / (CH / 8), c = (id % (CH / 8)) * 8;
-    const u4 v = r < nq ? *(const u4*)(src + r * ld + c) : (u4){0u, 0u, 0u, 0u};
-    *(u4*)(dst + r * CP + c) = v;
-  }
 }
 template <typename Hh, bool FFN>
 __device__ __forceinline__ void chain64_body(const ChainParams& p, const int tile, unsigned char* smem) {
@@ -390,14 +390,15 @@
 #define SEQ6(s) (FFN ? (s) : ((s) < 2 ? (s) : (s) + 16))
 #define AHEAD6(s) do { if ((s) + C6NB - 1 < NS) chain64_load_chunk<Hh>(ring[((s) + C6NB - 1) % C6NB], SEQ6((s) + C6NB - 1), p, w, lane, nj); } while (0)
   CH_MARK(0);
-  chain64_rows_in((const Hh*)p.inp + (long long)row0 * p.ld_in, p.ld_in, nq, sIn, tid);
-  chain64_rows_in((const Hh*)p.res + (long long)row0 * CH, CH, nq, sRes, tid);
+  ChainRows<C6ROWS, Hh> rows;
+  chain_rows_issue(rows, p, row0, nq, sIn, sRes, CP, tid);
   if (tid < CH) {
     sPar[tid] = p.ba[tid]; sPar[CH + tid] = p.g1[tid]; sPar[2 * CH + tid] = p.b1[tid];
     if (FFN) { sPar[3 * CH + tid] = p.bo2[tid]; sPar[4 * CH + tid] = p.g2[tid]; sPar[5 * CH + tid] = p.b2[tid]; }
   }
   if (FFN) { sPar[6 * CH + tid] = p.bi[tid]; sPar[6 * CH + 512 + tid] = p.bi[512 + tid]; }
   for (int i = tid; i < nj * 256; i += NWAVE * 64) sPar[6 * CH + CI + i] = p.bp[i];
+  chain_rows_store(rows, tid);
   h16x8<Hh> ring[C6NB][8];
 #pragma unroll
   for (int s = 0; s < C6NB - 1; ++s) chain64_load_chunk<Hh>(ring[s], SEQ6(s), p, w, lane, nj);
diff --git a/vln-magic_amd/csrc/common.hpp b/vln-magic_amd/csrc/common.hpp
--- a/vln-magic_amd/csrc/common.hpp
+++ b/vln-magic_amd/csrc/common.hpp
@@ -110,6 +110,27 @@
   for (int it = 0; it < NIT; ++it) {
     const int id = tid + (it0 + it) * nthr, r = id / im.cpr, c = (id - r * im.cpr) * VE;
     if (id < im.nchunk) *(rowvec<T>*)(im.s + r * im.pitch + c) = reg[it];
+  }
+}
+typedef unsigned u32x4 __attribute__((ext_vector_type(4)));
+template <int NIT, typename R>
+__device__ __forceinline__ void buf_stage_issue(u32x4 (&reg)[NIT], const R rsrc, const int cpr, const int ld, const int tid, const int nthr) {
+#pragma unroll
+  for (int it = 0; it < NIT; ++it) {
+    const int id = tid + it * nthr, r = id / cpr, c = (id - r * cpr) * 8;
+    reg[it] = __builtin_amdgcn_raw_buffer_load_b128(rsrc, (__mul24(r, ld) + c) * 2, 0, 16);
+  }
+}
+template <int NIT, typename T>
+__device__ __forceinline__ void buf_stage_store(const u32x4 (&reg)[NIT], T* s, T* own, const int pitch, const int cpr, const int nchunk, const int r0,
+                                                const int tid, const int nthr) {
+#pragma unroll
+  for (int it = 0; it < NIT; ++it) {
+    const int id = tid + it * nthr, r = id / cpr, c = (id - r * cpr) * 8;
+    if (id < nchunk) {
+      *(u32x4*)(s + r * pitch + c) = reg[it];
+      if (r >= r0 && r < r0 + 16) *(u32x4*)(own + (r - r0) * pitch + c) = reg[it];
+    }
   }
 }
 
diff --git a/vln-magic_amd/csrc/encoder.hip b/vln-magic_amd/csrc/encoder.hip
--- a/vln-magic_amd/csrc/encoder.hip
+++ b/vln-magic_amd/csrc/encoder.hip
@@ -123,7 +123,24 @@
   return __builtin_shufflevector(lo, hi, 0, 1, 2, 3, 4, 5, 6, 7);
 }
 
-template <int NRT, typename Hh>
+template <int NT>
+__device__ __forceinline__ void mask_words(unsigned (&km)[NT], const unsigned char* mask, const long long base, const int n, const int lane) {
+#pragma unroll
+  for (int j = 0; j < NT; ++j) {
+    const int key = j * 16 + (lane & 15);
+    km[j] = 1;
+    if (key < n && mask) km[j] = mask[base + key];
+  }
+}
+template <int NT>
+__device__ __forceinline__ void mask_bias(float (&bias)[NT], unsigned (&km)[NT]) {
+#pragma unroll
+  for (int j = 0; j < NT; ++j) asm volatile("" : "+v"(km[j]));
+#pragma unroll
+  for (int j = 0; j < NT; ++j) bias[j] = km[j] ? 0.f : -10000.0f;
+}
+
+template <int NRT, typename Hh, bool STAGED = false>
 __device__ __forceinline__ void enc_body(const EncParamsT<Hh>& p, const EncSegT<Hh>& sg, const int samp, unsigned char* smem) {
   typedef EncLay<NRT> LY;
   constexpr int RA = LY::RA, KR = LY::KR, PW = LY::PW;
@@ -139,7 +156,18 @@
   const long long row_base = (long long)samp * N;
   constexpr int ROWS = NRT * 16;
 
-  {
+  ENC_MARK(9);
+  float kbias[NRT];
+  if constexpr (STAGED) {
+    unsigned km[NRT];
+    mask_words<NRT>(km, sg.kmask, row_base, N, lane0);
+    constexpr int XIT = (ROWS * (EH / 8) + NWAVE * 64 - 1) / (NWAVE * 64);
+    const RowImg<Hh> iX = {sX, XS, sg.x + row_base * EH, EH, N, EH, EH / 8, ROWS * (EH / 8)};
+    rowvec<Hh> xr[XIT];
+    stage_issue<XIT>(xr, iX, 0, tid, NWAVE * 64);
+    stage_store<XIT>(xr, iX, 0, tid, NWAVE * 64);
+    mask_bias<NRT>(kbias, km);
+  } else {
     const Hh* x = sg.x + row_base * EH;
     for (int id = tid; id < ROWS * (EH / 8); id += NWAVE * 64) {
       const int r = id / (EH / 8), c = (id % (EH / 8)) * 8;
@@ -149,15 +177,15 @@
       if (r < N) v = *(const h16x8<Hh>*)(x + (long long)r * EH + c);
       *(h16x8<Hh>*)(sX + r * XS + c) = v;
     }
+#pragma unroll
+    for (int j = 0; j < NRT; ++j) {
+      const int key = j * 16 + (lane0 & 15);
+      kbias[j] = (key < N && sg.kmask && !sg.kmask[(long long)samp * N + key]) ? -10000.0f : 0.f;
+    }
   }
   DropDesc dd;
   dd.seed = p.seed;
-  float kbias[NRT];
-#pragma unroll
-  for (int j = 0; j < NRT; ++j) {
-    const int key = j * 16 + (lane0 & 15);
-    kbias[j] = (key < N && sg.kmask && !sg.kmask[(long long)samp * N + key]) ? -10000.0f : 0.f;
-  }
+  ENC_MARK(10);
   for (int l = 0; l < sg.nlayers; ++l) {
     const EncLayerT<Hh>& L = sg.L[l];
     int lane = lane0;
@@ -435,7 +463,6 @@
 #define RS_SS 84
 #define RS_PP 104
 #define RS_SPIN_MAX (1u << 21)
-typedef __attribute__((ext_vector_type(4))) unsigned u32x4;
 typedef __attribute__((address_space(1))) unsigned gu32_t;
 __device__ unsigned magic_enc_gave_up;
 __device__ __forceinline__ void enc_give_up(gu32_t* err) {
@@ -520,6 +547,16 @@
 #define RS_MARK(i) do { if (samp == 0 && tile == 0 && tid == 0 && &sg == &p.seg[0]) rs_ticks[l][i] = wall_clock64(); } while (0)
 #else
 #define RS_MARK(i)
+#endif
+#ifdef ENC_TIMING
+__device__ long long xrs_ticks[8][16];
+#define RS_ENTRY() do { if (samp == 0 && tile == 0 && tid == 0 && &sg == &p.seg[0]) rs_ticks[0][11] = wall_clock64(); } while (0)
+#define XRS_ENTRY() do { if (samp == 0 && tile == 0 && tid == 0 && &sg == &p.seg[0]) xrs_ticks[0][11] = wall_clock64(); } while (0)
+#define XRS_MARK(i) do { if (samp == 0 && tile == 0 && tid == 0 && &sg == &p.seg[0]) xrs_ticks[l][i] = wall_clock64(); } while (0)
+#else
+#define RS_ENTRY()
+#define XRS_ENTRY()
+#define XRS_MARK(i)
 #endif
 template <int NRT, typename Hh>
 __device__ __forceinline__ void enc_rs_body(const EncParamsT<Hh>& p, const EncSegT<Hh>& sg, const int samp, const int tile, unsigned* cnt,
@@ -542,6 +579,7 @@
   const long long row_base = (long long)samp * N;
   const int r0 = tile * 16, nq = min(16, N - r0);
   const long long row0 = row_base + r0;
+  RS_ENTRY();
   if (tid < XS / 8) {
     h16x8<Hh> zv;
 #pragma unroll
@@ -550,12 +588,8 @@
   }
   DropDesc dd;
   dd.seed = p.seed;
-  float kbias[NRT];
-#pragma unroll
-  for (int j = 0; j < NRT; ++j) {
-    const int key = j * 16 + (lane0 & 15);
-    kbias[j] = (key < N && sg.kmask && !sg.kmask[(long long)samp * N + key]) ? -10000.0f : 0.f;
-  }
+  unsigned km[NRT];
+  mask_words<NRT>(km, sg.kmask, (long long)samp * N, N, lane0);
   for (int l = 0; l < sg.nlayers; ++l) {
     const EncLayerT<Hh>& L = sg.L[l];
     int lane = lane0;
@@ -590,13 +624,13 @@
     {
       const Hh* x = (l == 0 ? sg.x : sg.L[l - 1].out) + row_base * EH;
       const auto rsrc = __builtin_amdgcn_make_buffer_rsrc((void*)x, 0, N * EH * 2, 0x00020000);
-      for (int id = tid; id < NRT * 16 * (EH / 8); id += NWAVE * 64) {
-        const int r = id / (EH / 8), c = (id % (EH / 8)) * 8;
-        const u32x4 v = __builtin_amdgcn_raw_buffer_load_b128(rsrc, (r * EH + c) * 2, 0, 16);
-        *(u32x4*)(sX + r * XS + c) = v;
-        if (r >= r0 && r < r0 + 16) *(u32x4*)(sO + (r - r0) * XS + c) = v;
-      }
-    }
+      constexpr int XIT = (NRT * 16 * (EH / 8) + NWAVE * 64 - 1) / (NWAVE * 64);
+      u32x4 xr[XIT];
+      buf_stage_issue<XIT>(xr, rsrc, EH / 8, EH, tid, NWAVE * 64);
+      buf_stage_store<XIT>(xr, sX, sO, XS, EH / 8, NRT * 16 * (EH / 8), r0, tid, NWAVE * 64);
+    }
+    float kbias[NRT];
+    mask_bias<NRT>(kbias, km);
     __syncthreads();
     RS_MARK(2);
     {
@@ -794,8 +828,8 @@
   switch (nt) {
     case 4: enc_rs_body<4>(p, sg, samp, tile, cnt, p.sync, enc_smem); break;
     case 5: enc_rs_body<5>(p, sg, samp, tile, cnt, p.sync, enc_smem); break;
-    case -3: enc_body<3>(p, sg, samp, enc_smem); break;
-    default: enc_body<2>(p, sg, samp, enc_smem); break;
+    case -3: enc_body<3, Hh, true>(p, sg, samp, enc_smem); break;
+    default: enc_body<2, Hh, true>(p, sg, samp, enc_smem); break;
   }
 }
 static size_t enc_rs_lds_bytes() { return (size_t)(80 * XS + 81 * XS + 80 * XS + 3 * 16 * XS) * 2 + 256 * sizeof(float); }
@@ -1089,6 +1123,15 @@
   }
 }
 
+template <typename Hh>
+__device__ __forceinline__ void ctx_frags(h16x8<Hh> (&a)[5], const Hh* cx, const int Nk, const int ks, const int lane) {
+#pragma unroll
+  for (int i = 0; i < 5; ++i) {
+    const int row = min(i * 16 + (lane & 15), Nk - 1);
+    a[i] = *(const h16x8<Hh>*)(cx + (__mul24(row, EH) + ks * 32 + 8 * (lane >> 4)));
+  }
+}
+
 template <int NRT, typename Hh>
 __device__ __forceinline__ void xenc_body(const XParamsT<Hh>& p, const XSegT<Hh>& sg, const int samp, unsigned char* smem) {
   constexpr int NKT = 5;
@@ -1439,6 +1482,7 @@
   const long long qbase = (long long)samp * Nq, kbase = (long long)samp * Nk;
   const int r0 = tile * 16, nq = min(16, Nq - r0);
   const long long row0 = qbase + r0;
+  XRS_ENTRY();
   if (tid < XS / 8) {
     h16x8<Hh> zv;
 #pragma unroll
@@ -1465,6 +1509,7 @@
     asm volatile("" : "+v"(lane));
     const int g = lane >> 4, c16 = lane & 15;
     const int colw = w * 16 + c16;
+    XRS_MARK(0);
     const float pb_q0 = L.bqkv[colw], pb_kv0 = L.bqkv[EH + (2 * w) * 16 + c16], pb_kv1 = L.bqkv[EH + (2 * w + 1) * 16 + c16];
     const float pb_ck0 = L.bkv[(2 * w) * 16 + c16], pb_ck1 = L.bkv[(2 * w + 1) * 16 + c16];
     float pb_ffn[4];
@@ -1492,6 +1537,7 @@
       __syncthreads();
     }
     {
+      XRS_MARK(1);
       const Hh* x = (l == 0 ? sg.x : sg.L[l - 1].out) + qbase * EH;
       const auto rsrc = __builtin_amdgcn_make_buffer_rsrc((void*)x, 0, Nq * EH * 2, 0x00020000);
       for (int id = tid; id < NRT * 16 * (EH / 8); id += NWAVE * 64) {
@@ -1502,6 +1548,7 @@
       }
     }
     __syncthreads();
+    XRS_MARK(2);
     {
       f32x4 acc[NRT][2], aq = (f32x4){0.f, 0.f, 0.f, 0.f};
 #pragma unroll
@@ -1557,8 +1604,12 @@
     for (int ct = 0; ct < 2; ++ct)
 #pragma unroll
       for (int ks = 0; ks < 4; ++ks) wck[ct][ks] = gfrag(L.Wkv, EH, (2 * w + ct) * 16, ks * 32, lane);
+    const Hh* cx = sg.cx + kbase * EH;
+    h16x8<Hh> ca[2][NKT];
+    ctx_frags(ca[0], cx, Nk, 0, lane);
     __syncthreads();
     copy_tile<false>(sA, XS, L.a + row0 * EH, EH, nq, EH, tid);
+    XRS_MARK(3);
     {
       f32x4 aq = (f32x4){0.f, 0.f, 0.f, 0.f};
 #pragma unroll
@@ -1568,15 +1619,13 @@
       f32x4 acc[NKT][2];
 #pragma unroll
       for (int i = 0; i < NKT; ++i) { acc[i][0] = (f32x4){0.f, 0.f, 0.f, 0.f}; acc[i][1] = (f32x4){0.f, 0.f, 0.f, 0.f}; }
-      const Hh* cx = sg.cx + kbase * EH;
 #pragma unroll
       for (int ks = 0; ks < 4; ++ks) {
+        if (ks < 3) ctx_frags(ca[(ks + 1) & 1], cx, Nk, ks + 1, lane);
 #pragma unroll
         for (int i = 0; i < NKT; ++i) {
-          const int row = min(i * 16 + c16, Nk - 1);
-          const h16x8<Hh> a = *(const h16x8<Hh>*)(cx + (long long)row * EH + ks * 32 + 8 * g);
-          acc[i][0] = mfma16(a, wck[0][ks], acc[i][0]);
-          acc[i][1] = mfma16(a, wck[1][ks], acc[i][1]);
+          acc[i][0] = mfma16(ca[ks & 1][i], wck[0][ks], acc[i][0]);
+          acc[i][1] = mfma16(ca[ks & 1][i], wck[1][ks], acc[i][1]);
         }
         KSTEP_FENCE();
       }
@@ -1598,6 +1647,7 @@
 #pragma unroll
       for (int ks = 0; ks < 4; ++ks) w1[ct][ks] = gfrag(L.W1, EH, (4 * w + ct) * 16, ks * 32, lane);
     __syncthreads();
+    XRS_MARK(4);
     copy_tile<false>(sQ, XS, L.q + row0 * EH, EH, nq, EH, tid);
     for (int kt = tile; kt * 16 < Nk; kt += ntile) {
       const int nr = min(16, Nk - kt * 16);
```

New measurement: 201,400, median of 6. No clear change (+0.4%).
